# microsoft/ctsTraffic

Hardware: AMD Instinct MI355X
Metric: GiB/s verified, 64 KiB buffers device-resident; % MI355X HBM roofline (higher is better)
Workload: dtype u8

## Files before the change

ctstraffic_amd/_lib.py:

```python
from __future__ import annotations

import ctypes
import os

try:
    import torch
except Exception:
    torch = None

_HERE = os.path.dirname(os.path.abspath(__file__))
LIB_PATH = os.environ.get("CTS_ENGINE_LIB") or os.path.join(_HERE, "libcts_engine.so")

CTS_OK = 0
CTS_E_INVALID = -1
CTS_E_HIP = -2
CTS_E_NOMEM = -3
CTS_E_NO_DEVICE = -4
CTS_E_UNAVAILABLE = -5
CTS_E_TIMEOUT = -6

PATTERN_PERIOD = 65536
UDP_DATA_HEADER_LENGTH = 26
STATUS_ERROR_DATA_DID_NOT_MATCH_BIT_PATTERN = 2147483644
STATUS_ERROR_TOO_MUCH_DATA_TRANSFERRED = 2147483645
STATUS_ERROR_NOT_ALL_DATA_TRANSFERRED = 2147483646
COUNTER_SHARDS = 64
ATTR_BLOCKS_PER_CU = 1
ATTR_NT_LOADS = 2
ATTR_SMALL_THRESHOLD = 3
ATTR_VERIFY_VARIANT = 4
ATTR_SMALL_BLOCKS_PER_CU = 5
ATTR_SMALL_VARIANT = 6
ATTR_FILL_BLOCKS_PER_CU = 7
ATTR_MS_VARIANT = 8
ATTR_SMALL_CHUNK = 9
ATTR_FILL_NT = 10
ATTR_SYNC_MAILBOX = 11


VERIFY_KERNEL_ID = 25


def verify_kernel_name(nontemporal: bool = True) -> str:
    return ("void cts::verify_wg_kernel<%s>(unsigned char const*, unsigned long, cts_buf_desc const*, unsigned int, "
            "cts_verify_result*, unsigned long*, unsigned int*, unsigned int)" % ("true" if nontemporal else "false"))


class CtsError(RuntimeError):
    def __init__(self, fn: str, status: int):
        super().__init__("%s failed: %s (%d)" % (fn, _status_string(status), status))
        self.status = status


class CtsCounters(ctypes.Structure):
    _fields_ = [
        ("bytes_checked", ctypes.c_uint64),
        ("bytes_ok", ctypes.c_uint64),
        ("buffers_checked", ctypes.c_uint64),
        ("buffers_failed", ctypes.c_uint64),
        ("mismatched_bytes", ctypes.c_uint64),
    ]

    def as_dict(self) -> dict:
        return {f: int(getattr(self, f)) for f, _ in self._fields_}


class CtsCountersEx(ctypes.Structure):
    _fields_ = CtsCounters._fields_ + [("connections_failed", ctypes.c_uint64)]

    def as_dict(self) -> dict:
        return {f: int(getattr(self, f)) for f, _ in self._fields_}


class CtsCountersRef(ctypes.Structure):
    _fields_ = [
        ("bytes_recv", ctypes.c_uint64),
        ("bytes_ok", ctypes.c_uint64),
        ("buffers_recv", ctypes.c_uint64),
        ("buffers_failed", ctypes.c_uint64),
        ("bytes_after_failure", ctypes.c_uint64),
        ("buffers_after_failure", ctypes.c_uint64),
    ]

    def as_dict(self) -> dict:
        return {f: int(getattr(self, f)) for f, _ in self._fields_}


class CtsCountersClose(ctypes.Structure):
    _fields_ = [
        ("connections_closed", ctypes.c_uint64),
        ("successful", ctypes.c_uint64),
        ("data_errors", ctypes.c_uint64),
        ("not_all_data", ctypes.c_uint64),
        ("too_much_data", ctypes.c_uint64),
        ("bytes_recv", ctypes.c_uint64),
    ]

    def as_dict(self) -> dict:
        return {f: int(getattr(self, f)) for f, _ in self._fields_}


class CtsCountersUdp(ctypes.Structure):
    _fields_ = [
        ("bits_received", ctypes.c_uint64),
        ("successful_frames", ctypes.c_uint64),
        ("dropped_frames", ctypes.c_uint64),
        ("duplicate_frames", ctypes.c_uint64),
        ("error_frames", ctypes.c_uint64),
        ("datagrams", ctypes.c_uint64),
    ]

    def as_dict(self) -> dict:
        return {f: int(getattr(self, f)) for f, _ in self._fields_}


class CtsCountersSent(ctypes.Structure):
    _fields_ = [
        ("bytes_sent", ctypes.c_uint64),
        ("buffers_sent", ctypes.c_uint64),
        ("connections_finished", ctypes.c_uint64),
        ("reserved0", ctypes.c_uint64),
        ("reserved1", ctypes.c_uint64),
        ("reserved2", ctypes.c_uint64),
    ]

    def as_dict(self) -> dict:
        return {f: int(getattr(self, f)) for f, _ in self._fields_}


class CtsAllreduceSetup(ctypes.Structure):
    _fields_ = [
        ("rccl_load_ms", ctypes.c_double),
        ("slots_ms", ctypes.c_double),
        ("comm_init_ms", ctypes.c_double),
        ("first_allreduce_ms", ctypes.c_double),
        ("devices", ctypes.c_uint32),
        ("prepared", ctypes.c_uint32),
        ("last_fold_us", ctypes.c_double),
        ("last_allreduce_us", ctypes.c_double),
        ("last_readback_us", ctypes.c_double),
        ("last_total_us", ctypes.c_double),
    ]

    def as_dict(self) -> dict:
        return {f: (float if t is ctypes.c_double else int)(getattr(self, f)) for f, t in self._fields_}


class CtsVerifyResult(ctypes.Structure):
    _fields_ = [
        ("first_mismatch", ctypes.c_uint32),
        ("mismatch_bytes", ctypes.c_uint32),
        ("expected", ctypes.c_uint8),
        ("actual", ctypes.c_uint8),
        ("pass_", ctypes.c_uint8),
        ("flags", ctypes.c_uint8),
    ]


assert ctypes.sizeof(CtsVerifyResult) == 12

_lib = None


def _status_string(status: int) -> str:
    try:
        return lib().cts_status_string(status).decode()
    except Exception:
        return "status"


def _declare(L: ctypes.CDLL) -> None:
    P = ctypes.c_void_p
    u32, u64, i32 = ctypes.c_uint32, ctypes.c_uint64, ctypes.c_int
    sigs = {
        "cts_version": ([], ctypes.c_char_p),
        "cts_status_string": ([i32], ctypes.c_char_p),
        "cts_pattern_byte": ([u64], ctypes.c_uint8),
        "cts_sender_buffer_size": ([u32], u64),
        "cts_shard_of": ([u32, u32], u32),
        "cts_engine_create": ([i32, ctypes.POINTER(P)], i32),
        "cts_engine_destroy": ([P], i32),
        "cts_engine_device": ([P], i32),
        "cts_engine_numa_node": ([P], i32),
        "cts_sender_buffer_fill": ([P, P, u32, P], i32),
        "cts_fill": ([P, P, u64, P, u32, u32, P], i32),
        "cts_verify": ([P, P, u64, P, u32, u32, P, P, P, u32, P], i32),
        "cts_verify_strided": ([P, P, u64, u32, P, u32, u32, u32, u32, P, P, P, u32, P], i32),
        "cts_verify_at": ([P, P, u64, P, u32, u32, u32, P, P, P, u32, P], i32),
        "cts_verify_strided_at": ([P, P, u64, u32, P, u32, u32, u32, u32, u32, P, P, P, u32, P], i32),
        "cts_refview_accumulate": ([P, u64, P, u32, u32, P, u32, P, P], i32),
        "cts_refview_accumulate_strided": ([P, u64, u32, P, u32, u32, u32, u32, P, u32, P, P], i32),
        "cts_counters_read_ref": ([P, P, ctypes.POINTER(CtsCountersRef), P], i32),
        "cts_counters_read_multi_ref": ([ctypes.POINTER(P), ctypes.POINTER(P), ctypes.POINTER(P), u32,
                                         ctypes.POINTER(CtsCountersRef)], i32),
        "cts_counters_allreduce_ref": ([ctypes.POINTER(P), ctypes.POINTER(P), ctypes.POINTER(P), u32,
                                        ctypes.POINTER(CtsCountersRef)], i32),
        "cts_refview_accumulate_conns": ([P, u64, P, u32, u32, P, u32, P, P, P], i32),
        "cts_refview_accumulate_conns_strided": ([P, u64, u32, P, u32, u32, u32, u32, P, u32, P, P, P], i32),
        "cts_conns_close": ([P, P, P, u32, P, P, u32, P, P, P], i32),
        "cts_conn_slots_rebase": ([P, P, u32, u32, P], i32),
        "cts_counters_read_close": ([P, P, ctypes.POINTER(CtsCountersClose), P], i32),
        "cts_counters_read_multi_close": ([ctypes.POINTER(P), ctypes.POINTER(P), ctypes.POINTER(P), u32,
                                           ctypes.POINTER(CtsCountersClose)], i32),
        "cts_counters_allreduce_close": ([ctypes.POINTER(P), ctypes.POINTER(P), ctypes.POINTER(P), u32,
                                          ctypes.POINTER(CtsCountersClose)], i32),
        "cts_ms_conn_init": ([P, u64, P], i32),
        "cts_media_stream_verify_status_at": ([P, P, u64, P, u32, u32, P, P, P, u32, P], i32),
        "cts_media_stream_conns_accumulate": ([P, u64, P, P, u32, u32, P, P, P, u64, u32, P, P], i32),
        "cts_media_stream_conns_render": ([P, P, u32, P, P, u32, P, P, P], i32),
        "cts_media_stream_conns_close": ([P, P, u32, P, P, P, u32, P, P, P], i32),
        "cts_counters_read_udp": ([P, P, ctypes.POINTER(CtsCountersUdp), P], i32),
        "cts_counters_read_multi_udp": ([ctypes.POINTER(P), ctypes.POINTER(P), ctypes.POINTER(P), u32,
                                         ctypes.POINTER(CtsCountersUdp)], i32),
        "cts_counters_allreduce_udp": ([ctypes.POINTER(P), ctypes.POINTER(P), ctypes.POINTER(P), u32,
                                        ctypes.POINTER(CtsCountersUdp)], i32),
        "cts_ms_server_init": ([P, P], i32),
        "cts_media_stream_servers_scratch_bytes": ([u32], ctypes.c_size_t),
        "cts_media_stream_servers_send": ([P, P, u64, u32, u64, u32, P, u32, P, u32, ctypes.c_int64, ctypes.c_int64,
                                           P, P, P, P, P, P, ctypes.c_size_t, P], i32),
        "cts_tcp_sender_init": ([u64, u32, P], i32),
        "cts_tcp_senders_scratch_bytes": ([u32], ctypes.c_size_t),
        "cts_tcp_senders_send": ([P, P, u64, u32, u64, u32, P, u32, u32, P, u32, P, P, P, P, P, ctypes.c_size_t, P],
                                 i32),
        "cts_counters_read_sent": ([P, P, ctypes.POINTER(CtsCountersSent), P], i32),
        "cts_counters_read_multi_sent": ([ctypes.POINTER(P), ctypes.POINTER(P), ctypes.POINTER(P), u32,
                                          ctypes.POINTER(CtsCountersSent)], i32),
        "cts_counters_allreduce_sent": ([ctypes.POINTER(P), ctypes.POINTER(P), ctypes.POINTER(P), u32,
                                         ctypes.POINTER(CtsCountersSent)], i32),
        "cts_counters_device_bytes": ([], ctypes.c_size_t),
        "cts_counters_reset": ([P, P, P], i32),
        "cts_counters_read": ([P, P, ctypes.POINTER(CtsCounters), P], i32),
        "cts_counters_read_multi": ([ctypes.POINTER(P), ctypes.POINTER(P), ctypes.POINTER(P), u32,
                                     ctypes.POINTER(CtsCounters)], i32),
        "cts_counters_allreduce": ([ctypes.POINTER(P), ctypes.POINTER(P), ctypes.POINTER(P), u32,
                                    ctypes.POINTER(CtsCounters)], i32),
        "cts_counters_allreduce_release": ([], i32),
        "cts_counters_read_ex": ([P, P, ctypes.POINTER(CtsCountersEx), P], i32),
        "cts_counters_read_multi_ex": ([ctypes.POINTER(P), ctypes.POINTER(P), ctypes.POINTER(P), u32,
                                        ctypes.POINTER(CtsCountersEx)], i32),
        "cts_counters_allreduce_ex": ([ctypes.POINTER(P), ctypes.POINTER(P), ctypes.POINTER(P), u32,
                                       ctypes.POINTER(CtsCountersEx)], i32),
        "cts_counters_allreduce_prepare": ([ctypes.POINTER(P), u32], i32),
        "cts_counters_allreduce_setup_times": ([ctypes.POINTER(CtsAllreduceSetup)], i32),
        "cts_verify_host": ([P, P, u32, u32, ctypes.POINTER(CtsVerifyResult)], i32),
        "cts_verify_mapped": ([P, P, u32, u32, ctypes.POINTER(CtsVerifyResult)], i32),
        "cts_mailbox_launches": ([P], u64),
        "cts_verify_host_batch": ([P, P, P, P, P, u32, P, ctypes.POINTER(CtsCounters)], i32),
        "cts_host_alloc": ([P, u64, ctypes.POINTER(P), ctypes.POINTER(P)], i32),
        "cts_host_free": ([P, P], i32),
        "cts_engine_set_attr": ([P, i32, i32], i32),
        "cts_engine_get_attr": ([P, i32, ctypes.POINTER(i32)], i32),
        "cts_engine_stream_create": ([P, ctypes.POINTER(P)], i32),
        "cts_engine_stream_destroy": ([P, P], i32),
        "cts_host_device_pointer": ([P, ctypes.POINTER(P)], i32),
    }
    for name, (argtypes, restype) in sigs.items():
        fn = getattr(L, name)
        fn.argtypes = argtypes
        fn.restype = restype
    from . import _pattern_abi, loopback, media_stream, status

    _pattern_abi.declare(L)
    media_stream.declare(L)
    loopback.declare(L)
    status.declare(L)


def lib() -> ctypes.CDLL:
    global _lib
    if _lib is None:
        if not os.path.exists(LIB_PATH):
            raise ImportError(
                "ctstraffic_amd: %s not built — run `make` or __graft_entry__.build() "
                "(the HIP engine has no CPU fallback)" % LIB_PATH
            )
        L = ctypes.CDLL(LIB_PATH, mode=ctypes.RTLD_GLOBAL)
        _declare(L)
        _lib = L
    return _lib


def check(fn: str, status: int) -> None:
    if status != CTS_OK:
        raise CtsError(fn, status)
```

ctstraffic_amd/csrc/cts_engine.cpp:

```cpp
#include <hip/hip_runtime_api.h>

#include <algorithm>
#include <atomic>
#include <cctype>
#include <chrono>
#include <condition_variable>
#include <cstdio>
#include <cstdlib>
#include <cstring>
#include <memory>
#include <mutex>
#include <new>
#include <string>
#include <system_error>
#include <thread>
#include <vector>

#include "cts_engine.h"
#include "cts_internal.hpp"
#include "cts_slices.hpp"

struct Mailbox;

struct cts_engine {
    int device = 0;
    cts::LaunchGeometry geo;
    std::mutex host_mu;
    hipStream_t stream = nullptr;
    uint8_t* stage = nullptr;
    size_t stage_cap = 0;
    cts_buf_desc* stage_desc = nullptr;
    cts_verify_result* stage_res = nullptr;
    void* batch_desc = nullptr;
    size_t batch_desc_cap = 0;
    void* batch_res = nullptr;
    size_t batch_res_cap = 0;
    void* batch_ctr = nullptr;
    int sync_mailbox = 1;
    struct HostStage {
        void* p = nullptr;
        size_t cap = 0;
    };
    std::mutex stage_pool_mu;
    std::vector<HostStage> stage_pool;
    std::unique_ptr<Mailbox> mail;
    std::mutex mail_init_mu;
};

namespace {

int env_int(const char* name, int dflt)
{
    const char* v = std::getenv(name);
    if (v == nullptr || *v == 0) return dflt;
    return std::atoi(v);
}

struct DeviceGuard {
    int prev = -1;
    bool ok = false;
    explicit DeviceGuard(int dev)
    {
        if (hipGetDevice(&prev) != hipSuccess) prev = -1;
        ok = (prev == dev) || (hipSetDevice(dev) == hipSuccess);
    }
    ~DeviceGuard()
    {
        if (prev >= 0) (void)hipSetDevice(prev);
    }
};

inline int hip_status(hipError_t e) { return e == hipSuccess ? CTS_OK : CTS_E_HIP; }

int host_alloc_mapped(size_t bytes, void** out)
{
    void* p = nullptr;
    if (hipHostMalloc(&p, bytes, hipHostMallocMapped | hipHostMallocPortable) != hipSuccess) return CTS_E_NOMEM;
    *out = p;
    return CTS_OK;
}

template <typename T>
T* device_view(T* host)
{
    void* d = nullptr;
    if (hipHostGetDevicePointer(&d, host, 0) != hipSuccess) return nullptr;
    return static_cast<T*>(d);
}

void pinned_free(cts_engine* e, void* p);

int ensure_pinned(cts_engine* e, void** p, size_t* cap, size_t bytes, size_t floor)
{
    if (*cap >= bytes && *p != nullptr) return CTS_OK;
    if (*p) pinned_free(e, *p);
    *p = nullptr;
    *cap = 0;
    size_t c = floor;
    while (c < bytes) c <<= 1;
    const int rc = host_alloc_mapped(c, p);
    if (rc != CTS_OK) return rc;
    *cap = c;
    return CTS_OK;
}

int ensure_stage(cts_engine* e, size_t bytes)
{
    void* p = e->stage;
    const int rc = ensure_pinned(e, &p, &e->stage_cap, bytes, 1u << 20);
    e->stage = static_cast<uint8_t*>(p);
    return rc;
}

}

struct Mailbox {
    cts_engine* e = nullptr;
    uint32_t nslots = 1024, groups = 8, per_group = 128;
    int exit_ms = 1000;
    uint64_t idle_ticks = 100000000ull;
    int idle_ms = 50;
    double timeout_s = 2.0;
    uint64_t delay_ticks = 0;
    cts::MailSlot* slots = nullptr;
    cts::MailSlot* dslots = nullptr;
    cts::MailPart* parts = nullptr;
    cts::MailPart* dparts = nullptr;
    hipStream_t stream = nullptr;
    hipEvent_t grid_done = nullptr;
    std::unique_ptr<std::atomic<uint64_t>[]> free_at;
    std::mutex mu;
    bool running = false, broken = false, quit = false;
    uint32_t paused = 0;
    uint64_t next[cts::kMailMaxGroups] = {};
    uint32_t busy[cts::kMailMaxGroups] = {};
    uint32_t outstanding = 0;
    std::chrono::steady_clock::time_point last_post;
    std::chrono::steady_clock::time_point last_used[cts::kMailMaxGroups];
    std::condition_variable cv;
    std::thread watchdog;
    std::atomic<uint64_t> launches{0};
    std::atomic<bool> broken_flag{false};

    ~Mailbox();

    int Init(cts_engine* eng)
    {
        e = eng;
        nslots = (uint32_t)std::max(16, env_int("CTS_MAILBOX_SLOTS", (int)nslots));
        groups = (uint32_t)std::min((int)cts::kMailMaxGroups, std::max(1, env_int("CTS_MAILBOX_GROUPS", (int)groups)));
        idle_ms = std::max(1, env_int("CTS_MAILBOX_IDLE_MS", idle_ms));
        exit_ms = std::max(40, env_int("CTS_MAILBOX_EXIT_MS", exit_ms));
        idle_ticks = (uint64_t)exit_ms * 100000ull;
        timeout_s = std::max(1, env_int("CTS_MAILBOX_TIMEOUT_MS", (int)(timeout_s * 1000))) / 1000.0;
        delay_ticks = (uint64_t)std::max(0, env_int("CTS_MAILBOX_DELAY_MS", 0)) * 100000ull;
        DeviceGuard g(e->device);
        if (!g.ok) return CTS_E_HIP;
        void* p = nullptr;
        per_group = (nslots + groups - 1) / groups;
        nslots = per_group * groups;
        if (hipHostMalloc(&p, sizeof(cts::MailSlot) * nslots,
                          hipHostMallocMapped | hipHostMallocPortable | hipHostMallocCoherent) != hipSuccess)
            return CTS_E_NOMEM;
        slots = static_cast<cts::MailSlot*>(p);
        std::memset(slots, 0, sizeof(cts::MailSlot) * nslots);
        if ((dslots = device_view(slots)) == nullptr) return CTS_E_HIP;
        const size_t pbytes = sizeof(cts::MailPart) * nslots * cts::kMailGroup;
        if (hipHostMalloc(&p, pbytes, hipHostMallocMapped | hipHostMallocPortable | hipHostMallocCoherent) !=
            hipSuccess)
            return CTS_E_NOMEM;
        parts = static_cast<cts::MailPart*>(p);
        std::memset(parts, 0, pbytes);
        if ((dparts = device_view(parts)) == nullptr) return CTS_E_HIP;
        if (hipStreamCreateWithFlags(&stream, hipStreamNonBlocking) != hipSuccess) {
            stream = nullptr;
            return CTS_E_HIP;
        }
        if (hipEventCreateWithFlags(&grid_done, hipEventDisableTiming) != hipSuccess) {
            grid_done = nullptr;
            return CTS_E_HIP;
        }
        free_at.reset(new (std::nothrow) std::atomic<uint64_t>[nslots]);
        if (!free_at) return CTS_E_NOMEM;
        ResetRings();
        last_post = std::chrono::steady_clock::now();
        try {
            watchdog = std::thread([this] { Watch(); });
        } catch (const std::system_error&) {
            return CTS_E_NOMEM;
        }
        return CTS_OK;
    }

    void ResetRings()
    {
        std::memset(slots, 0, sizeof(cts::MailSlot) * nslots);
        std::memset(parts, 0, sizeof(cts::MailPart) * nslots * cts::kMailGroup);
        for (uint32_t i = 0; i < nslots; ++i) free_at[i].store(i % per_group, std::memory_order_relaxed);
        for (uint32_t i = 0; i < cts::kMailMaxGroups; ++i) next[i] = busy[i] = 0;
    }

    bool DrainedLocked()
    {
        if (launches.load(std::memory_order_relaxed) == 0) return true;
        DeviceGuard g(e->device);
        return hipEventQuery(grid_done) == hipSuccess;
    }

    int LaunchLocked()
    {
        DeviceGuard g(e->device);
        if (!g.ok) return CTS_E_HIP;
        cts::MailStarts starts{};
        for (uint32_t i = 0; i < groups; ++i) starts.j[i] = next[i];
        const uint64_t delay = launches.load(std::memory_order_relaxed) == 0 ? delay_ticks : 0;
        if (cts::launch_mailbox(dslots, dparts, per_group, starts, groups, idle_ticks, stream, delay) != hipSuccess ||
            hipEventRecord(grid_done, stream) != hipSuccess)
            return CTS_E_HIP;
        running = true;
        launches.fetch_add(1, std::memory_order_relaxed);
        const auto now = std::chrono::steady_clock::now();
        for (uint32_t i = 0; i < groups; ++i) last_used[i] = now;
        return CTS_OK;
    }

    int Post(uint64_t ptr, uint32_t len, uint32_t expected, cts_verify_result* out, bool only_if_idle)
    {
        uint64_t js[cts::kMailMaxGroups];
        uint32_t g0 = 0, n = 1;
        {
            std::lock_guard<std::mutex> lk(mu);
            if (broken) {
                if (len == 0 || outstanding != 0 || !DrainedLocked()) return CTS_E_HIP;
                ResetRings();
                broken = false;
                broken_flag.store(false, std::memory_order_release);
            }
            if (len != 0 && paused != 0) return CTS_E_HIP;
            if (len == 0) {
                if (!running || (only_if_idle && outstanding != 0)) return CTS_OK;
                running = false;
                if (outstanding == 0 && DrainedLocked()) return CTS_OK;
                n = groups;
            } else {
                const auto now = std::chrono::steady_clock::now();
                if (running && now - last_post > std::chrono::milliseconds(exit_ms / 2)) {
                    DeviceGuard g(e->device);
                    if (hipEventQuery(grid_done) == hipSuccess) running = false;
                }
                if (!running) {
                    const int rc = LaunchLocked();
                    if (rc != CTS_OK) return rc;
                }
                for (uint32_t i = 1; i < groups; ++i)
                    if (busy[i] < busy[g0]) g0 = i;
                for (uint32_t i = 0; i < groups; ++i)
                    if (busy[i] == 0 && now - last_used[i] > std::chrono::milliseconds(exit_ms / 4)) {
                        g0 = i;
                        break;
                    }
                last_used[g0] = now;
            }
            for (uint32_t i = 0; i < n; ++i) {
                js[i] = next[g0 + i]++;
                ++busy[g0 + i];
            }
            ++outstanding;
            last_post = std::chrono::steady_clock::now();
        }
        int rc = CTS_OK;
        for (uint32_t i = 0; i < n && rc == CTS_OK; ++i) rc = Run(g0 + i, js[i], ptr, len, expected, out);
        std::lock_guard<std::mutex> lk(mu);
        if (rc != CTS_OK) {
            broken = true;
            broken_flag.store(true, std::memory_order_release);
            running = false;
        }
        for (uint32_t i = 0; i < n; ++i) --busy[g0 + i];
        --outstanding;
        return rc;
    }

    int Run(uint32_t g, uint64_t j, uint64_t ptr, uint32_t len, uint32_t expected, cts_verify_result* out)
    {
        const uint32_t k = g * per_group + (uint32_t)(j % per_group);
        const uint64_t t = j;
        while (free_at[k].load(std::memory_order_acquire) != t) {
            if (broken_flag.load(std::memory_order_acquire)) return CTS_E_HIP;
            std::this_thread::yield();
        }
        const uint32_t tag = (uint32_t)(t + 1);
        cts::mail_write(slots + k, (ptr & 0xFFFFFFFFFFFFull) | ((uint64_t)expected << 48), (uint64_t)len | ((uint64_t)tag << 32));
        const uint32_t np = cts::mail_parts(ptr, len);
        const cts::MailPart* const pr = parts + (size_t)k * cts::kMailGroup;
        const auto t_start = std::chrono::steady_clock::now();
        uint32_t first = 0xFFFFFFFFu, actual = 0;
        uint64_t count = 0;
        for (uint32_t i = 0; i < np; ++i) {
            uint64_t g0, g1;
            for (uint32_t spin = 0;; ++spin) {
                g0 = __atomic_load_n(&pr[i].g0, __ATOMIC_ACQUIRE);
                g1 = __atomic_load_n(&pr[i].g1, __ATOMIC_ACQUIRE);
                if ((uint32_t)(g0 >> 32) == tag && (uint32_t)(g1 >> 40) == (tag & 0xFFFFFFu)) break;
                if ((spin & 255u) == 255u) {
                    if (std::chrono::duration<double>(std::chrono::steady_clock::now() - t_start).count() > timeout_s)
                        return CTS_E_HIP;
                    std::this_thread::yield();
                }
            }
            if ((uint32_t)g0 < first) {
                first = (uint32_t)g0;
                actual = (uint32_t)(g1 >> 32) & 0xFFu;
            }
            count += (uint32_t)g1;
        }
        free_at[k].store(t + per_group, std::memory_order_release);
        if (out != nullptr && len != 0) {
            const bool pass = first == 0xFFFFFFFFu;
            out->first_mismatch = pass ? len : first;
            out->mismatch_bytes = (uint32_t)count;
            out->expected = pass ? 0 : cts_pattern_byte((uint64_t)expected + first);
            out->actual = pass ? 0 : (uint8_t)actual;
            out->pass = pass ? 1 : 0;
            out->flags = 0;
        }
        return CTS_OK;
    }

    int Stop(bool only_if_idle) { return Post(0, 0, 0, nullptr, only_if_idle); }

    void Pause()
    {
        {
            std::lock_guard<std::mutex> lk(mu);
            ++paused;
        }
        (void)Stop(false);
        const auto t0 = std::chrono::steady_clock::now();
        for (;;) {
            {
                std::lock_guard<std::mutex> lk(mu);
                if (DrainedLocked()) return;
            }
            if (std::chrono::duration<double>(std::chrono::steady_clock::now() - t0).count() > timeout_s) return;
            std::this_thread::yield();
        }
    }
    void Resume()
    {
        std::lock_guard<std::mutex> lk(mu);
        --paused;
    }

    void KeepaliveLocked(std::chrono::steady_clock::time_point now)
    {
        for (uint32_t g = 0; g < groups; ++g) {
            if (busy[g] != 0 || now - last_used[g] <= std::chrono::milliseconds(exit_ms / 4)) continue;
            const uint64_t t = next[g];
            const uint32_t k = g * per_group + (uint32_t)(t % per_group);
            if (free_at[k].load(std::memory_order_acquire) != t) continue;
            ++next[g];
            cts::mail_write(slots + k, 0, (uint64_t)cts::kMailSkip | ((uint64_t)(uint32_t)(t + 1) << 32));
            free_at[k].store(t + per_group, std::memory_order_release);
            last_used[g] = now;
        }
    }

    void Watch()
    {
        std::unique_lock<std::mutex> lk(mu);
        while (!quit) {
            cv.wait_for(lk, std::chrono::milliseconds(std::max(1, std::min(idle_ms / 2, exit_ms / 8))));
            if (quit || !running || broken) continue;
            const auto now = std::chrono::steady_clock::now();
            if (now - last_post < std::chrono::milliseconds(exit_ms / 2)) KeepaliveLocked(now);
            if (outstanding != 0) continue;
            if (now - last_post < std::chrono::milliseconds(idle_ms)) continue;
            lk.unlock();
            (void)Stop(true);
            lk.lock();
        }
    }
};

namespace {

std::mutex g_mail_reg_mu;
std::vector<Mailbox*> g_mail_reg;

class DeviceQuiesce {
public:
    explicit DeviceQuiesce(int device) : dev_(device), guard_(device), lk_(g_mail_reg_mu)
    {
        for (Mailbox* m : g_mail_reg)
            if (m->e->device == dev_) m->Pause();
    }
    ~DeviceQuiesce()
    {
        for (Mailbox* m : g_mail_reg)
            if (m->e->device == dev_) m->Resume();
    }
    DeviceQuiesce(const DeviceQuiesce&) = delete;
    DeviceQuiesce& operator=(const DeviceQuiesce&) = delete;

private:
    int dev_;
    DeviceGuard guard_;
    std::unique_lock<std::mutex> lk_;
};

int pinned_free_on(int device, void* p)
{
    DeviceQuiesce q(device);
    return hip_status(hipHostFree(p));
}

void pinned_free(cts_engine* e, void* p) { (void)pinned_free_on(e->device, p); }

int mailbox_of(cts_engine* e, Mailbox** out)
{
    std::lock_guard<std::mutex> lk(e->mail_init_mu);
    if (!e->mail) {
        std::unique_ptr<Mailbox> m(new (std::nothrow) Mailbox());
        if (!m) return CTS_E_NOMEM;
        const int rc = m->Init(e);
        if (rc != CTS_OK) return rc;
        {
            std::lock_guard<std::mutex> lk(g_mail_reg_mu);
            try {
                g_mail_reg.push_back(m.get());
            } catch (const std::bad_alloc&) {
                return CTS_E_NOMEM;
            }
        }
        e->mail = std::move(m);
    }
    *out = e->mail.get();
    return CTS_OK;
}

}

Mailbox::~Mailbox()
{
    if (e == nullptr) return;
    {
        std::lock_guard<std::mutex> lk(g_mail_reg_mu);
        g_mail_reg.erase(std::remove(g_mail_reg.begin(), g_mail_reg.end(), this), g_mail_reg.end());
    }
    {
        std::lock_guard<std::mutex> lk(mu);
        quit = true;
    }
    cv.notify_all();
    if (watchdog.joinable()) watchdog.join();
    (void)Stop(false);
    {
        DeviceGuard g(e->device);
        if (stream) {
            (void)hipStreamSynchronize(stream);
            (void)hipStreamDestroy(stream);
        }
        if (grid_done) (void)hipEventDestroy(grid_done);
    }
    if (parts == nullptr && slots == nullptr) return;
    DeviceQuiesce q(e->device);
    if (parts) (void)hipHostFree(parts);
    if (slots) (void)hipHostFree(slots);
}

const cts::LaunchGeometry& cts::engine_geometry(const cts_engine* e, int* device)
{
    if (device != nullptr) *device = e->device;
    return e->geo;
}

extern "C" {

const char* cts_version(void) { return "ctstraffic_amd 0.3.0 (gfx950)"; }

const char* cts_status_string(int status)
{
    switch (status) {
    case CTS_OK: return "ok";
    case CTS_E_INVALID: return "invalid argument";
    case CTS_E_HIP: return "HIP runtime error";
    case CTS_E_NOMEM: return "out of memory";
    case CTS_E_NO_DEVICE: return "no such HIP device";
    case CTS_E_UNAVAILABLE: return "runtime library unavailable (RCCL)";
    case CTS_E_TIMEOUT: return "timed out (nothing freed; retry)";
    default: return "unknown status";
    }
}

int cts_engine_create(int device, cts_engine** out)
{
    if (out == nullptr) return CTS_E_INVALID;
    *out = nullptr;
    int count = 0;
    if (hipGetDeviceCount(&count) != hipSuccess || count <= 0) return CTS_E_NO_DEVICE;
    if (device < 0 || device >= count) return CTS_E_NO_DEVICE;
    DeviceGuard g(device);
    if (!g.ok) return CTS_E_HIP;
    cts_engine* e = new (std::nothrow) cts_engine();
    if (e == nullptr) return CTS_E_NOMEM;
    e->device = device;
    int cus = 0;
    if (hipDeviceGetAttribute(&cus, hipDeviceAttributeMultiprocessorCount, device) == hipSuccess && cus > 0)
        e->geo.num_cus = cus;
    e->geo.blocks_per_cu = env_int("CTS_BLOCKS_PER_CU", e->geo.blocks_per_cu);
    e->geo.nontemporal = env_int("CTS_NT_LOADS", e->geo.nontemporal);
    e->geo.small_threshold = env_int("CTS_SMALL_THRESHOLD", e->geo.small_threshold);
    e->geo.small_blocks_per_cu = env_int("CTS_SMALL_BLOCKS_PER_CU", e->geo.small_blocks_per_cu);
    e->geo.fill_blocks_per_cu = env_int("CTS_FILL_BLOCKS_PER_CU", e->geo.fill_blocks_per_cu);
    e->geo.small_chunk = env_int("CTS_SMALL_CHUNK", e->geo.small_chunk);
    e->geo.fill_nt = env_int("CTS_FILL_NT", e->geo.fill_nt);
    e->geo.ring_fill_blocks_per_cu = env_int("CTS_RING_FILL_BLOCKS_PER_CU", e->geo.ring_fill_blocks_per_cu);
    e->sync_mailbox = env_int("CTS_SYNC_MAILBOX", e->sync_mailbox) ? 1 : 0;
    if (hipStreamCreateWithFlags(&e->stream, hipStreamNonBlocking) != hipSuccess) {
        delete e;
        return CTS_E_HIP;
    }
    void* p = nullptr;
    if (host_alloc_mapped(cts::kSliceMax * sizeof(cts_buf_desc), &p) != CTS_OK) {
        cts_engine_destroy(e);
        return CTS_E_NOMEM;
    }
    e->stage_desc = static_cast<cts_buf_desc*>(p);
    if (host_alloc_mapped(cts::kSliceMax * sizeof(cts_verify_result), &p) != CTS_OK) {
        cts_engine_destroy(e);
        return CTS_E_NOMEM;
    }
    e->stage_res = static_cast<cts_verify_result*>(p);
    *out = e;
    return CTS_OK;
}

int cts_engine_destroy(cts_engine* e)
{
    if (e == nullptr) return CTS_E_INVALID;
    e->mail.reset();
    {
        DeviceGuard g(e->device);
        if (e->stream) {
            (void)hipStreamSynchronize(e->stream);
            (void)hipStreamDestroy(e->stream);
        }
    }
    {
        DeviceQuiesce q(e->device);
        for (auto& st : e->stage_pool) (void)hipHostFree(st.p);
        e->stage_pool.clear();
        if (e->stage) (void)hipHostFree(e->stage);
        if (e->stage_desc) (void)hipHostFree(e->stage_desc);
        if (e->stage_res) (void)hipHostFree(e->stage_res);
        if (e->batch_desc) (void)hipHostFree(e->batch_desc);
        if (e->batch_res) (void)hipHostFree(e->batch_res);
        if (e->batch_ctr) (void)hipHostFree(e->batch_ctr);
    }
    delete e;
    return CTS_OK;
}

int cts_engine_device(const cts_engine* e) { return e ? e->device : CTS_E_INVALID; }

int cts_engine_numa_node(const cts_engine* e)
{
    if (e == nullptr) return -1;
    char bus[64] = {0};
    if (hipDeviceGetPCIBusId(bus, (int)sizeof(bus), e->device) != hipSuccess) return -1;
    std::string path = "/sys/bus/pci/devices/";
    for (const char* c = bus; *c; ++c) path += (char)std::tolower((unsigned char)*c);
    path += "/numa_node";
    FILE* f = std::fopen(path.c_str(), "r");
    if (f == nullptr) return -1;
    int node = -1;
    if (std::fscanf(f, "%d", &node) != 1) node = -1;
    std::fclose(f);
    return node;
}

int cts_engine_stream_create(cts_engine* e, void** stream)
{
    if (e == nullptr || stream == nullptr) return CTS_E_INVALID;
    DeviceGuard g(e->device);
    if (!g.ok) return CTS_E_HIP;
    hipStream_t s = nullptr;
    if (hipStreamCreateWithFlags(&s, hipStreamNonBlocking) != hipSuccess) return CTS_E_HIP;
    *stream = s;
    return CTS_OK;
}

int cts_engine_stream_destroy(cts_engine* e, void* stream)
{
    if (e == nullptr || stream == nullptr) return CTS_E_INVALID;
    DeviceGuard g(e->device);
    return hip_status(hipStreamDestroy(static_cast<hipStream_t>(stream)));
}

int cts_engine_set_attr(cts_engine* e, int attr, int value)
{
    if (e == nullptr) return CTS_E_INVALID;
    switch (attr) {
    case CTS_ATTR_BLOCKS_PER_CU:
        if (value < 1 || value > 64) return CTS_E_INVALID;
        e->geo.blocks_per_cu = value;
        return CTS_OK;
    case CTS_ATTR_NT_LOADS: e->geo.nontemporal = value ? 1 : 0; return CTS_OK;
    case CTS_ATTR_SMALL_THRESHOLD:
        if (value < 0) return CTS_E_INVALID;
        e->geo.small_threshold = value;
        return CTS_OK;
    case CTS_ATTR_VERIFY_VARIANT: return value == cts::kVerifyKernelId ? CTS_OK : CTS_E_INVALID;
    case CTS_ATTR_SMALL_VARIANT: return value == cts::kSmallKernelId ? CTS_OK : CTS_E_INVALID;
    case CTS_ATTR_MS_VARIANT: return value == cts::kMediaStreamKernelId ? CTS_OK : CTS_E_INVALID;
    case CTS_ATTR_SMALL_BLOCKS_PER_CU:
        if (value < 1 || value > 256) return CTS_E_INVALID;
        e->geo.small_blocks_per_cu = value;
        return CTS_OK;
    case CTS_ATTR_FILL_BLOCKS_PER_CU:
        if (value < 1 || value > 64) return CTS_E_INVALID;
        e->geo.fill_blocks_per_cu = value;
        return CTS_OK;
    case CTS_ATTR_SMALL_CHUNK:
        if (value < 0 || value > (1 << 24)) return CTS_E_INVALID;
        e->geo.small_chunk = value;
        return CTS_OK;
    case CTS_ATTR_SYNC_MAILBOX: e->sync_mailbox = value ? 1 : 0; return CTS_OK;
    case CTS_ATTR_FILL_NT:
        if (value < 0 || value > 2) return CTS_E_INVALID;
        e->geo.fill_nt = value;
        return CTS_OK;
    default: return CTS_E_INVALID;
    }
}

int cts_engine_get_attr(const cts_engine* e, int attr, int* value)
{
    if (e == nullptr || value == nullptr) return CTS_E_INVALID;
    switch (attr) {
    case CTS_ATTR_BLOCKS_PER_CU: *value = e->geo.blocks_per_cu; return CTS_OK;
    case CTS_ATTR_NT_LOADS: *value = e->geo.nontemporal; return CTS_OK;
    case CTS_ATTR_SMALL_THRESHOLD: *value = e->geo.small_threshold; return CTS_OK;
    case CTS_ATTR_VERIFY_VARIANT: *value = cts::kVerifyKernelId; return CTS_OK;
    case CTS_ATTR_SMALL_BLOCKS_PER_CU: *value = e->geo.small_blocks_per_cu; return CTS_OK;
    case CTS_ATTR_SMALL_VARIANT: *value = cts::kSmallKernelId; return CTS_OK;
    case CTS_ATTR_FILL_BLOCKS_PER_CU: *value = e->geo.fill_blocks_per_cu; return CTS_OK;
    case CTS_ATTR_MS_VARIANT: *value = cts::kMediaStreamKernelId; return CTS_OK;
    case CTS_ATTR_SMALL_CHUNK: *value = e->geo.small_chunk; return CTS_OK;
    case CTS_ATTR_FILL_NT: *value = e->geo.fill_nt; return CTS_OK;
    case CTS_ATTR_SYNC_MAILBOX: *value = e->sync_mailbox; return CTS_OK;
    default: return CTS_E_INVALID;
    }
}

int cts_sender_buffer_fill(cts_engine* e, void* dev_dst, uint32_t max_buffer_size, void* stream)
{
    if (e == nullptr || dev_dst == nullptr || ((uintptr_t)dev_dst & 15u) != 0) return CTS_E_INVALID;
    DeviceGuard g(e->device);
    if (!g.ok) return CTS_E_HIP;
    return hip_status(cts::launch_fill_span(static_cast<uint8_t*>(dev_dst), cts_sender_buffer_size(max_buffer_size), 0,
                                            static_cast<hipStream_t>(stream), e->geo));
}

int cts_fill(cts_engine* e, void* dev_arena, uint64_t arena_bytes, const cts_buf_desc* dev_descs, uint32_t n,
             uint32_t max_length_hint, void* stream)
{
    if (e == nullptr) return CTS_E_INVALID;
    if (n == 0) return CTS_OK;
    if (dev_arena == nullptr || dev_descs == nullptr || ((uintptr_t)dev_descs & 7u) != 0 || ((uintptr_t)dev_arena & 15u) != 0) return CTS_E_INVALID;
    DeviceGuard g(e->device);
    if (!g.ok) return CTS_E_HIP;
    return hip_status(cts::launch_fill(static_cast<uint8_t*>(dev_arena), arena_bytes, dev_descs, n, max_length_hint,
                                       static_cast<hipStream_t>(stream), e->geo));
}

static bool outputs_misaligned(const void* results, const void* counters, const void* conn_first_fail = nullptr)
{
    return ((uintptr_t)results & 3u) != 0 || ((uintptr_t)counters & 7u) != 0 || ((uintptr_t)conn_first_fail & 3u) != 0;
}

int cts_verify(cts_engine* e, const void* dev_arena, uint64_t arena_bytes, const cts_buf_desc* dev_descs, uint32_t n,
               uint32_t max_length_hint, cts_verify_result* dev_results, void* dev_counters,
               uint32_t* dev_conn_first_fail, uint32_t n_conns, void* stream)
{
    if (e == nullptr) return CTS_E_INVALID;
    if (n == 0) return CTS_OK;
    if (dev_arena == nullptr || dev_descs == nullptr || ((uintptr_t)dev_descs & 7u) != 0 || ((uintptr_t)dev_arena & 15u) != 0) return CTS_E_INVALID;
    if (dev_conn_first_fail == nullptr && n_conns != 0) return CTS_E_INVALID;
    if (outputs_misaligned(dev_results, dev_counters, dev_conn_first_fail)) return CTS_E_INVALID;
    DeviceGuard g(e->device);
    if (!g.ok) return CTS_E_HIP;
    return hip_status(cts::launch_verify(static_cast<const uint8_t*>(dev_arena), arena_bytes, dev_descs, n,
                                         max_length_hint, dev_results, static_cast<uint64_t*>(dev_counters),
                                         dev_conn_first_fail, n_conns, static_cast<hipStream_t>(stream), e->geo));
}

int cts_verify_strided(cts_engine* e, const void* dev_arena, uint64_t arena_bytes, uint32_t stride,
                       const uint32_t* dev_lengths, uint32_t n, uint32_t skip_head, uint32_t expected_offset,
                       uint32_t conn_index, cts_verify_result* dev_results, void* dev_counters,
                       uint32_t* dev_conn_first_fail, uint32_t n_conns, void* stream)
{
    if (e == nullptr) return CTS_E_INVALID;
    if (n == 0) return CTS_OK;
    if (dev_arena == nullptr || dev_lengths == nullptr || stride == 0 || arena_bytes < 16 ||
        ((uintptr_t)dev_arena & 15u) != 0 || ((uintptr_t)dev_lengths & 3u) != 0)
        return CTS_E_INVALID;
    if (expected_offset >= CTS_PATTERN_PERIOD) return CTS_E_INVALID;
    if (dev_conn_first_fail == nullptr && n_conns != 0) return CTS_E_INVALID;
    if (outputs_misaligned(dev_results, dev_counters, dev_conn_first_fail)) return CTS_E_INVALID;
    DeviceGuard g(e->device);
    if (!g.ok) return CTS_E_HIP;
    return hip_status(cts::launch_verify_strided(static_cast<const uint8_t*>(dev_arena), arena_bytes, stride, dev_lengths, n,
                                                 skip_head, expected_offset, conn_index, dev_results,
                                                 static_cast<uint64_t*>(dev_counters), dev_conn_first_fail, n_conns,
                                                 static_cast<hipStream_t>(stream), e->geo));
}

int cts_media_stream_fill(cts_engine* e, void* dev_arena, uint64_t arena_bytes, const cts_buf_desc* dev_descs,
                          const cts_datagram_header* dev_headers, uint32_t n, void* stream)
{
    if (e == nullptr) return CTS_E_INVALID;
    if (n == 0) return CTS_OK;
    if (dev_arena == nullptr || dev_descs == nullptr || ((uintptr_t)dev_descs & 7u) != 0 || dev_headers == nullptr ||
        ((uintptr_t)dev_headers & 7u) != 0)
        return CTS_E_INVALID;
    DeviceGuard g(e->device);
    if (!g.ok) return CTS_E_HIP;
    return hip_status(cts::launch_media_stream_fill(static_cast<uint8_t*>(dev_arena), arena_bytes, dev_descs,
                                                    dev_headers, n, static_cast<hipStream_t>(stream), e->geo));
}

int cts_media_stream_fill_strided(cts_engine* e, void* dev_arena, uint64_t arena_bytes, uint32_t stride,
                                  const uint32_t* dev_lengths, const cts_datagram_header* dev_headers, uint32_t n,
                                  void* stream)
{
    if (e == nullptr) return CTS_E_INVALID;
    if (n == 0) return CTS_OK;
    if (dev_arena == nullptr || ((uintptr_t)dev_arena & 15u) != 0 || dev_lengths == nullptr ||
        ((uintptr_t)dev_lengths & 3u) != 0 || dev_headers == nullptr || ((uintptr_t)dev_headers & 7u) != 0 ||
        stride < 32u || (stride & 15u) != 0 || stride > (1u << 20))
        return CTS_E_INVALID;
    DeviceGuard g(e->device);
    if (!g.ok) return CTS_E_HIP;
    return hip_status(cts::launch_media_stream_fill_strided(static_cast<uint8_t*>(dev_arena), arena_bytes, stride,
                                                            dev_lengths, dev_headers, n,
                                                            static_cast<hipStream_t>(stream), e->geo));
}

int cts_media_stream_verify(cts_engine* e, const void* dev_arena, uint64_t arena_bytes, const cts_buf_desc* dev_descs,
                            uint32_t n, cts_datagram_record* dev_records, cts_verify_result* dev_results,
                            void* dev_counters, void* stream)
{
    if (e == nullptr) return CTS_E_INVALID;
    if (n == 0) return CTS_OK;
    if (dev_arena == nullptr || dev_descs == nullptr || ((uintptr_t)dev_descs & 7u) != 0 || ((uintptr_t)dev_arena & 15u) != 0) return CTS_E_INVALID;
    if (outputs_misaligned(dev_results, dev_counters, dev_records)) return CTS_E_INVALID;
    DeviceGuard g(e->device);
    if (!g.ok) return CTS_E_HIP;
    return hip_status(cts::launch_media_stream_verify(static_cast<const uint8_t*>(dev_arena), arena_bytes, dev_descs,
                                                      n, dev_records, dev_results,
                                                      static_cast<uint64_t*>(dev_counters),
                                                      static_cast<hipStream_t>(stream), e->geo));
}

int cts_media_stream_verify_strided(cts_engine* e, const void* dev_arena, uint64_t arena_bytes, uint32_t stride,
                                    const uint32_t* dev_lengths, uint32_t n, cts_datagram_record* dev_records,
                                    cts_verify_result* dev_results, void* dev_counters, void* stream)
{
    if (e == nullptr) return CTS_E_INVALID;
    if (n == 0) return CTS_OK;
    if (dev_arena == nullptr || dev_lengths == nullptr || ((uintptr_t)dev_lengths & 3u) != 0 ||
        ((uintptr_t)dev_arena & 15u) != 0 || arena_bytes < 16u || stride == 0)
        return CTS_E_INVALID;
    if (outputs_misaligned(dev_results, dev_counters, dev_records)) return CTS_E_INVALID;
    DeviceGuard g(e->device);
    if (!g.ok) return CTS_E_HIP;
    return hip_status(cts::launch_media_stream_verify_strided(static_cast<const uint8_t*>(dev_arena), arena_bytes, stride,
                                                              dev_lengths, n, dev_records, dev_results,
                                                              static_cast<uint64_t*>(dev_counters),
                                                              static_cast<hipStream_t>(stream), e->geo));
}

int cts_media_stream_verify_status(cts_engine* e, const void* dev_arena, uint64_t arena_bytes,
                                   const cts_buf_desc* dev_descs, uint32_t n, cts_datagram_status* dev_status,
                                   void* dev_counters, void* stream)
{
    if (e == nullptr) return CTS_E_INVALID;
    if (n == 0) return CTS_OK;
    if (dev_arena == nullptr || dev_descs == nullptr || ((uintptr_t)dev_descs & 7u) != 0 || ((uintptr_t)dev_arena & 15u) != 0 ||
        outputs_misaligned(dev_status, dev_counters))
        return CTS_E_INVALID;
    DeviceGuard g(e->device);
    if (!g.ok) return CTS_E_HIP;
    return hip_status(cts::launch_media_stream_status(static_cast<const uint8_t*>(dev_arena), arena_bytes, dev_descs,
                                                      nullptr, 0u, n, dev_status, static_cast<uint64_t*>(dev_counters),
                                                      static_cast<hipStream_t>(stream), e->geo));
}

int cts_media_stream_verify_strided_status(cts_engine* e, const void* dev_arena, uint64_t arena_bytes, uint32_t stride,
                                           const uint32_t* dev_lengths, uint32_t n, cts_datagram_status* dev_status,
                                           void* dev_counters, void* stream)
{
    if (e == nullptr) return CTS_E_INVALID;
    if (n == 0) return CTS_OK;
    if (dev_arena == nullptr || dev_lengths == nullptr || ((uintptr_t)dev_lengths & 3u) != 0 ||
        ((uintptr_t)dev_arena & 15u) != 0 || arena_bytes < 16u || stride == 0 || outputs_misaligned(dev_status, dev_counters))
        return CTS_E_INVALID;
    DeviceGuard g(e->device);
    if (!g.ok) return CTS_E_HIP;
    return hip_status(cts::launch_media_stream_status(static_cast<const uint8_t*>(dev_arena), arena_bytes, nullptr,
                                                      dev_lengths, stride, n, dev_status,
                                                      static_cast<uint64_t*>(dev_counters),
                                                      static_cast<hipStream_t>(stream), e->geo));
}

static int media_stream_frames(cts_engine* e, const void* dev_arena, uint64_t arena_bytes, const cts_buf_desc* dev_descs,
                               uint32_t stride, const uint32_t* dev_lengths, uint32_t n, const cts_frame_window* w,
                               void* dev_totals, uint64_t* dev_frame_bytes, void* dev_counters, void* stream)
{
    if (e == nullptr || w == nullptr || dev_totals == nullptr || ((uintptr_t)dev_totals & 7u) != 0 ||
        (w->frames != 0 && (dev_frame_bytes == nullptr || ((uintptr_t)dev_frame_bytes & 7u) != 0)))
        return CTS_E_INVALID;
    if (n != 0 && (dev_arena == nullptr || ((uintptr_t)dev_arena & 15u) != 0 || outputs_misaligned(nullptr, dev_counters)))
        return CTS_E_INVALID;
    if (n != 0 && dev_descs == nullptr &&
        (dev_lengths == nullptr || ((uintptr_t)dev_lengths & 3u) != 0 || arena_bytes < 16u || stride == 0))
        return CTS_E_INVALID;
    if (n != 0 && dev_descs != nullptr && ((uintptr_t)dev_descs & 7u) != 0) return CTS_E_INVALID;
    DeviceGuard g(e->device);
    if (!g.ok) return CTS_E_HIP;
    return hip_status(cts::launch_media_stream_frames(static_cast<const uint8_t*>(dev_arena), arena_bytes, dev_descs,
                                                      dev_lengths, stride, n, *w, static_cast<uint64_t*>(dev_totals),
                                                      dev_frame_bytes, static_cast<uint64_t*>(dev_counters),
                                                      static_cast<hipStream_t>(stream), e->geo));
}

int cts_media_stream_verify_frames(cts_engine* e, const void* dev_arena, uint64_t arena_bytes,
                                   const cts_buf_desc* dev_descs, uint32_t n, const cts_frame_window* window,
                                   void* dev_totals, uint64_t* dev_frame_bytes, void* dev_counters, void* stream)
{
    if (n != 0 && dev_descs == nullptr) return CTS_E_INVALID;
    return media_stream_frames(e, dev_arena, arena_bytes, dev_descs, 0u, nullptr, n, window, dev_totals,
                               dev_frame_bytes, dev_counters, stream);
}

int cts_media_stream_verify_strided_frames(cts_engine* e, const void* dev_arena, uint64_t arena_bytes, uint32_t stride,
                                           const uint32_t* dev_lengths, uint32_t n, const cts_frame_window* window,
                                           void* dev_totals, uint64_t* dev_frame_bytes, void* dev_counters,
                                           void* stream)
{
    if (n != 0 && dev_lengths == nullptr) return CTS_E_INVALID;
    return media_stream_frames(e, dev_arena, arena_bytes, nullptr, stride, dev_lengths, n, window, dev_totals,
                               dev_frame_bytes, dev_counters, stream);
}

size_t cts_counters_device_bytes(void) { return (size_t)CTS_COUNTER_SHARDS * cts::kCounterSlots * sizeof(uint64_t); }

int cts_counters_reset(cts_engine* e, void* dev_counters, void* stream)
{
    if (e == nullptr || dev_counters == nullptr) return CTS_E_INVALID;
    DeviceGuard g(e->device);
    if (!g.ok) return CTS_E_HIP;
    return hip_status(hipMemsetAsync(dev_counters, 0, cts_counters_device_bytes(), static_cast<hipStream_t>(stream)));
}

int cts_counters_read_ex(cts_engine* e, const void* dev_counters, cts_counters_ex* out, void* stream)
{
    if (e == nullptr || dev_counters == nullptr || out == nullptr) return CTS_E_INVALID;
    DeviceGuard g(e->device);
    if (!g.ok) return CTS_E_HIP;
    uint64_t h[CTS_COUNTER_SHARDS * cts::kCounterSlots];
    hipStream_t s = static_cast<hipStream_t>(stream);
    if (hipMemcpyAsync(h, dev_counters, cts_counters_device_bytes(), hipMemcpyDeviceToHost, s) != hipSuccess)
        return CTS_E_HIP;
    if (hipStreamSynchronize(s) != hipSuccess) return CTS_E_HIP;
    uint64_t v[cts::kCounterCount] = {};
    for (uint32_t sh = 0; sh < CTS_COUNTER_SHARDS; ++sh)
        for (int k = 0; k < cts::kCounterCount; ++k) v[k] += h[sh * cts::kCounterSlots + k];
    *out = cts::counters_ex_of(v);
    return CTS_OK;
}

int cts_counters_read(cts_engine* e, const void* dev_counters, cts_counters* out, void* stream)
{
    if (out == nullptr) return CTS_E_INVALID;
    cts_counters_ex x{};
    const int rc = cts_counters_read_ex(e, dev_counters, &x, stream);
    if (rc == CTS_OK) *out = cts::counters_of(x);
    return rc;
}

int cts_host_alloc(cts_engine* e, uint64_t bytes, void** host_ptr, void** dev_view)
{
    if (e == nullptr || host_ptr == nullptr || bytes == 0) return CTS_E_INVALID;
    DeviceGuard g(e->device);
    if (!g.ok) return CTS_E_HIP;
    void* p = nullptr;
    const int rc = host_alloc_mapped((size_t)((bytes + 15u) & ~(uint64_t)15u), &p);
    if (rc != CTS_OK) return rc;
    *host_ptr = p;
    if (dev_view != nullptr) {
        void* d = nullptr;
        if (hipHostGetDevicePointer(&d, p, 0) != hipSuccess) {
            (void)pinned_free_on(e->device, p);
            *host_ptr = nullptr;
            return CTS_E_HIP;
        }
        *dev_view = d;
    }
    return CTS_OK;
}

int cts_host_free(cts_engine* e, void* host_ptr)
{
    if (e == nullptr || host_ptr == nullptr) return CTS_E_INVALID;
    return pinned_free_on(e->device, host_ptr);
}

int cts_host_device_pointer(void* host_ptr, void** dev_view)
{
    if (host_ptr == nullptr || dev_view == nullptr) return CTS_E_INVALID;
    void* d = nullptr;
    if (hipHostGetDevicePointer(&d, host_ptr, 0) != hipSuccess) return CTS_E_INVALID;
    *dev_view = d;
    return CTS_OK;
}

int cts_verify_host(cts_engine* e, const void* host_buf, uint32_t len, uint32_t expected_offset, cts_verify_result* out)
{
    if (e == nullptr || out == nullptr || (host_buf == nullptr && len != 0)) return CTS_E_INVALID;
    if (expected_offset >= CTS_PATTERN_PERIOD) return CTS_E_INVALID;
    if (e->sync_mailbox) {
        cts_engine::HostStage st;
        {
            std::lock_guard<std::mutex> lk(e->stage_pool_mu);
            if (!e->stage_pool.empty()) {
                st = e->stage_pool.back();
                e->stage_pool.pop_back();
            }
        }
        int rc = ensure_pinned(e, &st.p, &st.cap, (size_t)len + 16, 64u << 10);
        const uint8_t* dev = rc == CTS_OK ? device_view(static_cast<uint8_t*>(st.p)) : nullptr;
        if (rc == CTS_OK && dev == nullptr) rc = CTS_E_HIP;
        if (rc == CTS_OK) {
            if (len) std::memcpy(st.p, host_buf, len);
            rc = cts_verify_mapped(e, dev, len, expected_offset, out);
        }
        if (st.p != nullptr) {
            bool pooled = false;
            {
                std::lock_guard<std::mutex> lk(e->stage_pool_mu);
                try {
                    e->stage_pool.push_back(st);
                    pooled = true;
                } catch (const std::bad_alloc&) {
                }
            }
            if (!pooled) pinned_free(e, st.p);
        }
        return rc;
    }
    std::lock_guard<std::mutex> lk(e->host_mu);
    DeviceGuard g(e->device);
    if (!g.ok) return CTS_E_HIP;
    int rc = ensure_stage(e, (size_t)len + 16);
    if (rc != CTS_OK) return rc;
    if (len) std::memcpy(e->stage, host_buf, len);
    uint32_t slice_len = 0;
    const uint32_t ns = cts::slice_plan(0, len, expected_offset, 0, e->stage_desc, &slice_len);
    const uint8_t* arena = device_view(e->stage);
    const cts_buf_desc* dd = device_view(e->stage_desc);
    cts_verify_result* dr = device_view(e->stage_res);
    if (!arena || !dd || !dr) return CTS_E_HIP;
    hipError_t err = cts::launch_verify(arena, e->stage_cap, dd, ns, slice_len, dr, nullptr, nullptr, 0, e->stream,
                                        e->geo);
    if (err == hipSuccess) err = hipStreamSynchronize(e->stream);
    if (err != hipSuccess) return CTS_E_HIP;
    *out = cts::slice_merge(e->stage_res, ns, slice_len, len);
    return CTS_OK;
}

int cts_verify_host_batch(cts_engine* e, const void* const* bufs, const uint32_t* lens, const uint32_t* expected,
                          const uint32_t* skip_heads, uint32_t n, cts_verify_result* results, cts_counters* counters)
{
    if (e == nullptr) return CTS_E_INVALID;
    if (n == 0) return CTS_OK;
    if (bufs == nullptr || lens == nullptr || expected == nullptr || results == nullptr) return CTS_E_INVALID;
    std::lock_guard<std::mutex> lk(e->host_mu);
    DeviceGuard g(e->device);
    if (!g.ok) return CTS_E_HIP;
    uint64_t total = 0;
    for (uint32_t i = 0; i < n; ++i) {
        if (bufs[i] == nullptr && lens[i] != 0) return CTS_E_INVALID;
        total += ((uint64_t)lens[i] + 15u) & ~(uint64_t)15u;
    }
    int rc = ensure_stage(e, (size_t)total + 16);
    if (rc != CTS_OK) return rc;
    if ((rc = ensure_pinned(e, &e->batch_desc, &e->batch_desc_cap, sizeof(cts_buf_desc) * n, 4096)) != CTS_OK) return rc;
    if ((rc = ensure_pinned(e, &e->batch_res, &e->batch_res_cap, sizeof(cts_verify_result) * n, 4096)) != CTS_OK) return rc;
    if (counters && e->batch_ctr == nullptr &&
        (rc = host_alloc_mapped(cts_counters_device_bytes(), &e->batch_ctr)) != CTS_OK)
        return rc;
    void* const pres = e->batch_res;
    void* const pctr = counters ? e->batch_ctr : nullptr;
    cts_buf_desc* hd = static_cast<cts_buf_desc*>(e->batch_desc);
    uint64_t off = 0;
    uint32_t maxlen = 0;
    for (uint32_t i = 0; i < n; ++i) {
        if (lens[i]) std::memcpy(e->stage + off, bufs[i], lens[i]);
        hd[i].byte_offset = off;
        hd[i].length = lens[i];
        hd[i].expected_pattern_offset = expected[i];
        hd[i].conn_index = i;
        hd[i].skip_head = skip_heads ? skip_heads[i] : 0u;
        maxlen = lens[i] > maxlen ? lens[i] : maxlen;
        off += ((uint64_t)lens[i] + 15u) & ~(uint64_t)15u;
    }
    if (pctr) std::memset(pctr, 0, cts_counters_device_bytes());
    hipError_t err = cts::launch_verify(device_view(e->stage), e->stage_cap, device_view(hd), n, maxlen,
                                        device_view(static_cast<cts_verify_result*>(pres)),
                                        pctr ? device_view(static_cast<uint64_t*>(pctr)) : nullptr, nullptr, 0,
                                        e->stream, e->geo);
    if (err == hipSuccess) err = hipStreamSynchronize(e->stream);
    if (err == hipSuccess) {
        std::memcpy(results, pres, sizeof(cts_verify_result) * n);
        if (counters) {
            const uint64_t* h = static_cast<const uint64_t*>(pctr);
            for (uint32_t sh = 0; sh < CTS_COUNTER_SHARDS; ++sh) {
                counters->bytes_checked += h[sh * cts::kCounterSlots + cts::kBytesChecked];
                counters->bytes_ok += h[sh * cts::kCounterSlots + cts::kBytesOk];
                counters->buffers_checked += h[sh * cts::kCounterSlots + cts::kBuffersChecked];
                counters->buffers_failed += h[sh * cts::kCounterSlots + cts::kBuffersFailed];
                counters->mismatched_bytes += h[sh * cts::kCounterSlots + cts::kMismatchedBytes];
            }
        }
    }
    return err == hipSuccess ? CTS_OK : CTS_E_HIP;
}

int cts_verify_mapped(cts_engine* e, const void* dev_buf, uint32_t len, uint32_t expected_offset,
                      cts_verify_result* out)
{
    if (e == nullptr || out == nullptr || (dev_buf == nullptr && len != 0)) return CTS_E_INVALID;
    if (expected_offset >= CTS_PATTERN_PERIOD) return CTS_E_INVALID;
    if (len == 0) {
        *out = cts_verify_result{0, 0, 0, 0, 1, 0};
        return CTS_OK;
    }
    Mailbox* m = nullptr;
    const int rc = mailbox_of(e, &m);
    if (rc != CTS_OK) return rc;
    if (m->Post(reinterpret_cast<uint64_t>(dev_buf), len, expected_offset, out, false) == CTS_OK) return CTS_OK;
    std::lock_guard<std::mutex> lk(e->host_mu);
    DeviceGuard g(e->device);
    if (!g.ok) return CTS_E_HIP;
    const uint64_t d = reinterpret_cast<uintptr_t>(dev_buf) & 15u;
    uint32_t slice_len = 0;
    const uint32_t ns = cts::slice_plan(d, len, expected_offset, 0, e->stage_desc, &slice_len);
    const cts_buf_desc* dd = device_view(e->stage_desc);
    cts_verify_result* dr = device_view(e->stage_res);
    if (!dd || !dr) return CTS_E_HIP;
    hipError_t err = cts::launch_verify(static_cast<const uint8_t*>(dev_buf) - d, d + len, dd, ns, slice_len, dr,
                                        nullptr, nullptr, 0, e->stream, e->geo);
    if (err == hipSuccess) err = hipStreamSynchronize(e->stream);
    if (err != hipSuccess) return CTS_E_HIP;
    *out = cts::slice_merge(e->stage_res, ns, slice_len, len);
    return CTS_OK;
}

uint64_t cts_mailbox_launches(const cts_engine* e)
{
    return (e != nullptr && e->mail) ? e->mail->launches.load(std::memory_order_relaxed) : 0;
}

}
```

ctstraffic_amd/csrc/cts_fill.hip:

```cpp
#include <hip/hip_runtime.h>

#include "cts_chunks.hpp"
#include "cts_launch.hpp"

namespace cts {


__device__ __forceinline__ void store_chunk_bytes(uint8_t* dst, const u32x4& e, uint32_t b0, uint32_t b1)
{
#pragma unroll
    for (uint32_t w = 0; w < 4u; ++w) {
        const uint32_t lo = b0 > 4u * w ? b0 - 4u * w : 0u, hi = b1 < 4u * w + 4u ? (b1 > 4u * w ? b1 - 4u * w : 0u) : 4u;
        if (lo >= hi) continue;
        uint8_t* q = dst + 4u * w;
        const uint32_t v = e[w];
        if (lo == 0u && hi == 4u) {
            *reinterpret_cast<uint32_t*>(q) = v;
            continue;
        }
        uint32_t b = lo;
        if ((b & 1u) && b < hi) {
            q[b] = (uint8_t)(v >> (8u * b));
            ++b;
        }
        if (b + 2u <= hi) {
            *reinterpret_cast<uint16_t*>(q + b) = (uint16_t)(v >> (8u * b));
            b += 2u;
        }
        if (b < hi) q[b] = (uint8_t)(v >> (8u * b));
    }
}

template <bool NTS = false>
__device__ __forceinline__ void fill_chunk(u32x4* a0, uint32_t c, uint32_t nchunks, uint32_t q0, uint32_t lo,
                                           uint32_t hi_last)
{
    const u32x4 e = expected_chunk((q0 + 16u * c) & 0xFFFFu, q0 & 1u);
    const bool first_c = (c == 0u);
    const bool last_c = (c == nchunks - 1u);
    const uint32_t b0 = first_c ? lo : 0u;
    const uint32_t b1 = last_c ? hi_last : 16u;
    if (b0 == 0u && b1 == 16u) {
        if constexpr (NTS) __builtin_nontemporal_store(e, a0 + c);
        else a0[c] = e;
    } else {
        store_chunk_bytes(reinterpret_cast<uint8_t*>(a0 + c), e, b0, b1);
    }
}

template <int TEAM, int U, bool EVEN, bool NTS>
__device__ __forceinline__ void fill_whole_rounds(u32x4* p, uint32_t nchunks, uint32_t q0, uint32_t lane)
{
    const uint32_t sh = q0 & 1u;
    typedef u32x4 __attribute__((address_space(1)))* gstore_ptr;
    uint32_t cb = 0;
    for (; cb + (uint32_t)(TEAM * U) <= nchunks; cb += (uint32_t)(TEAM * U)) {
        const uint32_t k = ((q0 + 16u * (cb + lane)) & 0xFFFFu) >> 1;
        const uint32_t B = __umul24(k, 0x10001u) + 0x10000u;
        const gstore_ptr g = (gstore_ptr)(p + cb + lane);
#pragma unroll
        for (int u = 0; u < U; ++u) {
            const u32x4 e = expected_step<TEAM, U, EVEN>(B, u, sh);
            if constexpr (NTS) __builtin_nontemporal_store(e, g + u * TEAM);
            else g[u * TEAM] = e;
        }
    }
    if (cb < nchunks) {
        const __amdgpu_buffer_rsrc_t r = __builtin_amdgcn_make_buffer_rsrc(p, (short)0, (int)(nchunks * 16u), 0x00020000);
        const uint32_t k = ((q0 + 16u * (cb + lane)) & 0xFFFFu) >> 1;
        const uint32_t B = __umul24(k, 0x10001u) + 0x10000u;
#pragma unroll
        for (int u = 0; u < U; ++u)
            __builtin_amdgcn_raw_buffer_store_b128(expected_step<TEAM, U, EVEN>(B, u, sh), r,
                                                   (cb + (uint32_t)(u * TEAM) + lane) * 16u, 0u, NTS ? 2 : 0);
    }
}

template <int TEAM, int FU, bool NTS>
__device__ __forceinline__ void fill_one(uint8_t* arena, uint64_t arena_bytes, const cts_buf_desc& d, uint32_t lane)
{
    if (desc_bad(d, arena_bytes)) return;
    const uint32_t len = d.length - d.skip_head;
    if (len == 0) return;
    uint8_t* sp = arena + d.byte_offset + d.skip_head;
    const uint32_t lo = (uint32_t)((uintptr_t)sp & 15u);
    const uint32_t nchunks = (uint32_t)(((uint64_t)lo + len + 15u) >> 4);
    const uint32_t hi_last = (uint32_t)((uint64_t)lo + len - 16ull * (nchunks - 1u));
    const uint32_t q0 = (d.expected_pattern_offset - lo) & 0xFFFFu;
    u32x4* p = reinterpret_cast<u32x4*>(sp - lo);
    if (__builtin_amdgcn_readfirstlane((lo == 0u && hi_last == 16u && nchunks < kGiantChunks) ? 1u : 0u)) {
        if (__builtin_amdgcn_readfirstlane(q0 & 1u) == 0u) fill_whole_rounds<TEAM, FU, true, NTS>(p, nchunks, q0, lane);
        else fill_whole_rounds<TEAM, FU, false, NTS>(p, nchunks, q0, lane);
        return;
    }
    for (uint32_t c = lane; c < nchunks; c += TEAM) fill_chunk<NTS>(p, c, nchunks, q0, lo, hi_last);
}

template <int TEAM, bool NTS = false>
__global__ void __launch_bounds__(kBlock) fill_kernel(uint8_t* __restrict__ arena, uint64_t arena_bytes,
                                                      const cts_buf_desc* __restrict__ descs, uint32_t n)
{
#include "cts_fill_team_loop.hpp"
}

constexpr uint32_t kFillPiece = 8192;
constexpr int kPieceBatch = 16;

struct PieceJob {
    uint64_t base;
    uint32_t q0;
    uint32_t cb, ce;
    uint32_t nchunks, lo, hi_last;
    uint32_t kind;
};

template <uint32_t PIECE>
__device__ __forceinline__ PieceJob decode_piece(uint8_t* arena, uint64_t arena_bytes, const cts_buf_desc* descs,
                                                 uint64_t v, uint64_t total, uint32_t ppb, bool mine)
{
    constexpr uint32_t kChunks = PIECE / 16;
    PieceJob j{};
    if (!mine || v >= total) return j;
    const uint32_t i = (uint32_t)(v / ppb), pc = (uint32_t)(v - (uint64_t)i * ppb);
    const cts_buf_desc d = descs[i];
    if (desc_bad(d, arena_bytes) || d.length == d.skip_head) return j;
    const uint32_t len = d.length - d.skip_head;
    const uint64_t sp = (uint64_t)(uintptr_t)arena + d.byte_offset + d.skip_head;
    j.lo = (uint32_t)(sp & 15u);
    j.nchunks = (uint32_t)(((uint64_t)j.lo + len + 15u) >> 4);
    j.hi_last = (uint32_t)((uint64_t)j.lo + len - 16ull * (j.nchunks - 1u));
    j.q0 = (d.expected_pattern_offset - j.lo) & 0xFFFFu;
    j.base = sp - j.lo;
    const uint64_t cb = (uint64_t)pc * kChunks;
    if (cb >= j.nchunks) return j;
    j.cb = (uint32_t)cb;
    j.ce = pc + 1u == ppb ? j.nchunks : (uint32_t)(cb + kChunks < j.nchunks ? cb + kChunks : j.nchunks);
    j.kind = (j.lo == 0u && j.hi_last == 16u) ? 1u : 2u;
    return j;
}

__device__ __forceinline__ uint32_t lane_u32(uint32_t x, int m) { return (uint32_t)__builtin_amdgcn_readlane((int)x, m); }

template <bool NTS, uint32_t PIECE = kFillPiece, int BATCH = kPieceBatch>
__global__ void __launch_bounds__(kBlock) fill_pieces_kernel(uint8_t* __restrict__ arena, uint64_t arena_bytes,
                                                             const cts_buf_desc* __restrict__ descs, uint32_t n,
                                                             uint32_t ppb)
{
#include "cts_fill_pieces_loop.hpp"
}

__global__ void __launch_bounds__(kBlock) fill_span_kernel(uint8_t* __restrict__ dst, uint64_t bytes, uint32_t e)
{
    const uint32_t lo = (uint32_t)((uintptr_t)dst & 15u);
    const uint32_t nchunks = (uint32_t)((lo + bytes + 15u) >> 4);
    const uint32_t hi_last = (uint32_t)(lo + bytes - 16ull * (nchunks - 1u));
    const uint32_t q0 = (e - lo) & 0xFFFFu;
    u32x4* p = reinterpret_cast<u32x4*>(dst - lo);
    for (uint32_t c = blockIdx.x * kBlock + threadIdx.x; c < nchunks; c += gridDim.x * kBlock)
        fill_chunk(p, c, nchunks, q0, lo, hi_last);
}

template <bool NTS>
__device__ __forceinline__ void ms_fill_one(uint8_t* arena, uint64_t arena_bytes, const cts_buf_desc& d, uint64_t seq,
                                            uint64_t qpc, uint64_t qpf, uint32_t lane)
{
    if (d.length < CTS_UDP_DATA_HEADER_LENGTH || d.byte_offset > arena_bytes ||
        arena_bytes - d.byte_offset < (uint64_t)d.length)
        return;
    uint8_t* dg = arena + d.byte_offset;
    if (__builtin_amdgcn_readfirstlane(((uintptr_t)dg & 15u) == 0u ? 1u : 0u)) {
        const uint32_t nchunks = (d.length + 15u) >> 4;
        const uint32_t hi_last = d.length - 16u * (nchunks - 1u);
        u32x4* p = reinterpret_cast<u32x4*>(dg);
        for (uint32_t c = lane; c < nchunks; c += 64u) {
            u32x4 e = expected_chunk((16u * c - CTS_UDP_DATA_HEADER_LENGTH) & 0xFFFFu, 0u);
            if (c == 0u)
                e = u32x4{(uint32_t)(seq << 16), (uint32_t)(seq >> 16), (uint32_t)(seq >> 48) | (uint32_t)(qpc << 16),
                          (uint32_t)(qpc >> 16)};
            else if (c == 1u)
                e = u32x4{(uint32_t)(qpc >> 48) | (uint32_t)(qpf << 16), (uint32_t)(qpf >> 16),
                          (uint32_t)(qpf >> 48) | (e[2] & 0xFFFF0000u), e[3]};
            if (c == nchunks - 1u && hi_last != 16u) {
                store_chunk_bytes(reinterpret_cast<uint8_t*>(p + c), e, 0u, hi_last);
            } else {
                if constexpr (NTS) __builtin_nontemporal_store(e, p + c);
                else p[c] = e;
            }
        }
        return;
    }
    if (lane < CTS_UDP_DATA_HEADER_LENGTH) {
        uint8_t b = 0;
        if (lane >= 2u && lane < 10u) b = (uint8_t)(seq >> (8 * (lane - 2u)));
        else if (lane >= 10u && lane < 18u) b = (uint8_t)(qpc >> (8 * (lane - 10u)));
        else if (lane >= 18u) b = (uint8_t)(qpf >> (8 * (lane - 18u)));
        dg[lane] = b;
    }
    const uint32_t len = d.length - CTS_UDP_DATA_HEADER_LENGTH;
    if (len == 0) return;
    uint8_t* sp = dg + CTS_UDP_DATA_HEADER_LENGTH;
    const uint32_t lo = (uint32_t)((uintptr_t)sp & 15u);
    const uint32_t nchunks = (uint32_t)(((uint64_t)lo + len + 15u) >> 4);
    const uint32_t hi_last = (uint32_t)((uint64_t)lo + len - 16ull * (nchunks - 1u));
    const uint32_t q0 = (0u - lo) & 0xFFFFu;
    u32x4* p = reinterpret_cast<u32x4*>(sp - lo);
    for (uint32_t c = lane; c < nchunks; c += 64u) fill_chunk<NTS>(p, c, nchunks, q0, lo, hi_last);
}

constexpr uint32_t kFillBatch = kBlock;

template <bool NTS>
__global__ void __launch_bounds__(kBlock)
    fill_batched_kernel(uint8_t* __restrict__ arena, uint64_t arena_bytes, const cts_buf_desc* __restrict__ descs,
                        const cts_datagram_header* __restrict__ headers, uint32_t n)
{
    constexpr uint32_t WAVES = kBlock / 64;
    __shared__ cts_buf_desc ds[kFillBatch];
    __shared__ cts_datagram_header hs[kFillBatch];
    const uint32_t lane = threadIdx.x & 63u;
    const uint32_t wave = (uint32_t)__builtin_amdgcn_readfirstlane(threadIdx.x >> 6);
    const uint32_t per_wg = (uint32_t)(((uint64_t)n + gridDim.x - 1u) / gridDim.x);
    const uint64_t g0 = (uint64_t)blockIdx.x * per_wg;
    const uint64_t g1 = g0 + per_wg < n ? g0 + per_wg : n;
    for (uint64_t d0 = g0; d0 < g1; d0 += kFillBatch) {
        const uint32_t nb = (uint32_t)(g1 - d0 < kFillBatch ? g1 - d0 : kFillBatch);
        __syncthreads();
        if (threadIdx.x < nb) {
            ds[threadIdx.x] = descs[d0 + threadIdx.x];
            hs[threadIdx.x] = headers[d0 + threadIdx.x];
        }
        __syncthreads();
        const uint32_t q = (nb + WAVES - 1u) / WAVES;
        const uint32_t t1 = (wave + 1u) * q < nb ? (wave + 1u) * q : nb;
        for (uint32_t t = wave * q; t < t1; ++t) {
            const cts_datagram_header h = hs[t];
            ms_fill_one<NTS>(arena, arena_bytes, ds[t], (uint64_t)h.sequence_number, (uint64_t)h.qpc, (uint64_t)h.qpf,
                             lane);
        }
    }
}


constexpr uint32_t kRingBatch = 512;

struct RingHeader {
    uint64_t seq, qpc, qpf;
};

__device__ __forceinline__ u32x4 datagram_chunk(uint32_t c, const u32x4& pattern, uint64_t seq, uint64_t qpc,
                                                uint64_t qpf)
{
    if (c == 0u)
        return u32x4{(uint32_t)(seq << 16), (uint32_t)(seq >> 16), (uint32_t)(seq >> 48) | (uint32_t)(qpc << 16),
                     (uint32_t)(qpc >> 16)};
    if (c == 1u)
        return u32x4{(uint32_t)(qpc >> 48) | (uint32_t)(qpf << 16), (uint32_t)(qpf >> 16),
                     (uint32_t)(qpf >> 48) | (pattern[2] & 0xFFFF0000u), pattern[3]};
    return pattern;
}

__device__ __forceinline__ u32x4 header_lanes(u32x4 e, uint32_t lane, uint32_t l0, const RingHeader& h)
{
    if (lane == l0) {
        e = u32x4{(uint32_t)(h.seq << 16), (uint32_t)(h.seq >> 16), (uint32_t)(h.seq >> 48) | (uint32_t)(h.qpc << 16),
                  (uint32_t)(h.qpc >> 16)};
    } else if (lane == l0 + 1u) {
        e[0] = (uint32_t)(h.qpc >> 48) | (uint32_t)(h.qpf << 16);
        e[1] = (uint32_t)(h.qpf >> 16);
        e[2] = (uint32_t)(h.qpf >> 48) | (e[2] & 0xFFFF0000u);
    }
    return e;
}

template <bool NTS>
__device__ __forceinline__ void ring_chunk_checked(u32x4* ring, uint64_t k, uint64_t j, uint32_t c, uint32_t len,
                                                   const RingHeader& h, uint32_t stride, uint64_t arena_bytes)
{
    if (len < CTS_UDP_DATA_HEADER_LENGTH || len > stride || 16u * c >= len || j * stride + len > arena_bytes) return;
    const u32x4 e = datagram_chunk(c, expected_chunk((16u * c - CTS_UDP_DATA_HEADER_LENGTH) & 0xFFFFu, 0u), h.seq,
                                   h.qpc, h.qpf);
    if (16u * c + 16u > len) {
        store_chunk_bytes(reinterpret_cast<uint8_t*>(ring + k), e, 0u, len - 16u * c);
    } else {
        if constexpr (NTS) __builtin_nontemporal_store(e, ring + k);
        else ring[k] = e;
    }
}

template <bool NTS, bool SCALAR>
__global__ void __launch_bounds__(kBlock)
    media_stream_fill_ring_kernel(uint8_t* __restrict__ arena, uint64_t arena_bytes, uint32_t stride,
                                  const uint32_t* __restrict__ lengths, const cts_datagram_header* __restrict__ headers,
                                  uint32_t n, uint32_t full_slots)
{
    constexpr uint32_t WAVES = kBlock / 64;
    __shared__ RingHeader hs[kRingBatch];
    __shared__ uint32_t ls[kRingBatch];
    const uint32_t lane = threadIdx.x & 63u;
    const uint32_t wave = (uint32_t)__builtin_amdgcn_readfirstlane(threadIdx.x >> 6);
    const uint32_t cps = stride >> 4;
    const uint32_t per_wg = (uint32_t)(((uint64_t)n + gridDim.x - 1u) / gridDim.x);
    const uint64_t g0 = (uint64_t)blockIdx.x * per_wg;
    const uint64_t g1 = g0 + per_wg < n ? g0 + per_wg : n;
    u32x4* const ring = reinterpret_cast<u32x4*>(arena);
    for (uint64_t d0 = g0; d0 < g1; d0 += kRingBatch) {
        const uint32_t nb = (uint32_t)(g1 - d0 < kRingBatch ? g1 - d0 : kRingBatch);
        __syncthreads();
        for (uint32_t t = threadIdx.x; t < nb; t += kBlock) {
            const cts_datagram_header h = headers[d0 + t];
            hs[t] = RingHeader{(uint64_t)h.sequence_number, (uint64_t)h.qpc, (uint64_t)h.qpf};
            ls[t] = lengths[d0 + t];
        }
        __syncthreads();
#include "cts_ring_store_loop.hpp"
    }
}


__device__ __forceinline__ uint32_t ms_server_want(const cts_ms_server_state* __restrict__ servers, uint32_t c,
                                                   uint32_t n_conns, uint32_t stride, uint32_t& code)
{
    code = CTS_MS_SERVER_SKIPPED;
    if (c >= n_conns) return 0u;
    if (servers[c].finished != 0u) {
        code = CTS_MS_SERVER_ENDED;
        return 0u;
    }
    if (servers[c].datagram_max_size > stride) return 0u;
    code = CTS_MS_SERVER_SENT;
    return servers[c].datagrams_per_frame;
}

__device__ __forceinline__ uint64_t tile_scan_exclusive(uint64_t v, uint64_t* wsum, uint64_t& total)
{
    const uint32_t lane = threadIdx.x & 63u, wave = threadIdx.x >> 6;
    uint64_t inc = v;
#pragma unroll
    for (uint32_t off = 1; off < 64u; off <<= 1) {
        const uint64_t u = (uint64_t)__shfl_up((unsigned long long)inc, off, 64);
        if (lane >= off) inc += u;
    }
    if (lane == 63u) wsum[wave] = inc;
    __syncthreads();
    uint64_t base = 0;
    total = 0;
#pragma unroll
    for (uint32_t w = 0; w < (uint32_t)kBlock / 64u; ++w) {
        if (w < wave) base += wsum[w];
        total += wsum[w];
    }
    __syncthreads();
    return base + inc - v;
}

static_assert(kMsServerTile == (uint32_t)kBlock, "one listed connection per thread of a tile");

__global__ void __launch_bounds__(kBlock)
    ms_server_sums(const uint32_t* __restrict__ ids, uint32_t n, const cts_ms_server_state* __restrict__ servers,
                   uint32_t n_conns, uint32_t stride, uint64_t* __restrict__ sums)
{
    __shared__ uint64_t wsum[kBlock / 64];
    const uint64_t i = (uint64_t)blockIdx.x * kMsServerTile + threadIdx.x;
    uint32_t code;
    const uint64_t want = i < n ? ms_server_want(servers, ids[i], n_conns, stride, code) : 0u;
    const uint64_t s = wave_sum64(want);
    if ((threadIdx.x & 63u) == 0u) wsum[threadIdx.x >> 6] = s;
    __syncthreads();
    if (threadIdx.x == 0u) {
        uint64_t t = 0;
#pragma unroll
        for (int w = 0; w < kBlock / 64; ++w) t += wsum[w];
        sums[blockIdx.x] = t;
    }
}

__global__ void __launch_bounds__(kBlock)
    ms_server_scan(uint64_t* __restrict__ sums, uint64_t tiles, uint64_t* __restrict__ prefix_total,
                   uint32_t* __restrict__ tick)
{
    __shared__ uint64_t wsum[kBlock / 64];
    uint64_t carry = 0;
    for (uint64_t base = 0; base < tiles; base += kBlock) {
        const uint64_t t = base + threadIdx.x;
        const uint64_t v = t < tiles ? sums[t] : 0u;
        uint64_t total;
        const uint64_t ex = tile_scan_exclusive(v, wsum, total);
        if (t < tiles) sums[t] = carry + ex;
        carry += total;
    }
    if (threadIdx.x == 0u) *prefix_total = carry;
    if (threadIdx.x < sizeof(cts_ms_server_tick) / 4u) tick[threadIdx.x] = 0u;
}

__global__ void __launch_bounds__(kBlock)
    ms_server_apply(const uint32_t* __restrict__ ids, uint32_t n, cts_ms_server_state* __restrict__ servers,
                    uint32_t n_conns, uint32_t stride, uint32_t capacity, const uint64_t* __restrict__ sums,
                    uint64_t* __restrict__ prefix, uint32_t* __restrict__ codes, cts_ms_server_tick* __restrict__ tick,
                    uint64_t* __restrict__ udp)
{
    __shared__ uint64_t wsum[kBlock / 64];
    __shared__ uint64_t ctr[kBlock / 64][kCounterCount];
    __shared__ uint32_t red[kBlock / 64][5];
    zero_counters<kBlock / 64>(ctr);
    const uint64_t i = (uint64_t)blockIdx.x * kMsServerTile + threadIdx.x;
    uint32_t code = CTS_MS_SERVER_SENT, c = 0u;
    uint64_t want = 0;
    if (i < n) {
        c = ids[i];
        want = ms_server_want(servers, c, n_conns, stride, code);
    }
    uint64_t total;
    const uint64_t p = sums[blockIdx.x] + tile_scan_exclusive(want, wsum, total);
    uint64_t bytes = 0;
    uint32_t datagrams = 0, sent = 0, finished = 0, no_room = 0, skipped = 0;
    if (i < n) {
        prefix[i] = p;
        if (code != CTS_MS_SERVER_SENT) {
            skipped = 1u;
        } else if (p + want > (uint64_t)capacity) {
            no_room = 1u;
            code = CTS_MS_SERVER_NO_ROOM;
        } else {
            cts_ms_server_state* e = servers + c;
            bytes = e->frame_size_bytes;
            datagrams = (uint32_t)want;
            sent = 1u;
            e->bits_sent += 8u * bytes;
            e->datagrams_sent += want;
            const int64_t next = e->current_frame + 1;
            e->current_frame = next;
            if (next > e->final_frame) {
                e->finished = 1u;
                finished = 1u;
                code = CTS_MS_SERVER_FINISHED;
            }
        }
        if (codes != nullptr) codes[i] = code;
    }
    bytes = wave_sum64(bytes);
    datagrams = wave_sum(datagrams);
    sent = wave_sum(sent);
    finished = wave_sum(finished);
    no_room = wave_sum(no_room);
    skipped = wave_sum(skipped);
    const uint32_t wave = threadIdx.x >> 6;
    if ((threadIdx.x & 63u) == 0u) {
        ctr[wave][0] = 8u * bytes;
        ctr[wave][kCounterCount - 1] = datagrams;
        red[wave][0] = datagrams;
        red[wave][1] = sent;
        red[wave][2] = finished;
        red[wave][3] = no_room;
        red[wave][4] = skipped;
    }
    flush_counters<kBlock / 64>(udp, ctr);
    if (threadIdx.x < 5u) {
        uint32_t s = 0;
#pragma unroll
        for (int w = 0; w < kBlock / 64; ++w) s += red[w][threadIdx.x];
        uint32_t* const words = &tick->datagrams;
        if (s) atomicAdd(words + threadIdx.x, s);
    } else if (threadIdx.x == 5u) {
        uint64_t s = 0;
#pragma unroll
        for (int w = 0; w < kBlock / 64; ++w) s += ctr[w][0];
        if (s) atomicAdd((unsigned long long*)&tick->bytes, (unsigned long long)(s / 8u));
    }
}

__device__ __forceinline__ uint64_t ms_server_listed(const uint64_t* __restrict__ prefix, uint64_t lo, uint64_t hi,
                                                     uint64_t g)
{
    while (hi - lo > 1u) {
        const uint64_t mid = lo + (hi - lo) / 2u;
        if (prefix[mid] <= g) lo = mid;
        else hi = mid;
    }
    return lo;
}

__device__ __forceinline__ uint32_t ms_server_length(uint32_t F, uint32_t M, uint32_t k, uint32_t j)
{
    const uint32_t r = F % (M != 0u ? M : 1u);
    const bool tiny = r != 0u && r <= CTS_UDP_DATA_HEADER_LENGTH;
    if (j + 1u == k) return r == 0u ? M : (tiny && k > 1u ? CTS_UDP_DATA_HEADER_LENGTH + 1u : r);
    if (j + 2u == k && tiny) return M - (CTS_UDP_DATA_HEADER_LENGTH + 1u - r);
    return M;
}

template <bool NTS, bool SCALAR>
__global__ void __launch_bounds__(kBlock)
    ms_server_fill(uint8_t* __restrict__ ring_base, uint64_t arena_bytes, uint32_t stride, uint64_t first_slot,
                          const uint32_t* __restrict__ ids, uint32_t n,
                          const cts_ms_server_state* __restrict__ servers, const uint64_t* __restrict__ prefix,
                          const cts_ms_server_tick* __restrict__ tick, uint64_t qpc, uint64_t qpf,
                          cts_buf_desc* __restrict__ descs, uint32_t* __restrict__ lengths, uint32_t full_slots,
                          uint32_t capacity, uint32_t n_conns)
{
    constexpr uint32_t WAVES = kBlock / 64;
    __shared__ RingHeader hs[kRingBatch];
    __shared__ uint32_t ls[kRingBatch];
    __shared__ uint64_t ps[kRingBatch + 1];
    __shared__ uint64_t first_listed;
    const uint32_t total = tick->datagrams < capacity ? tick->datagrams : capacity;
    if (total == 0u) return;
    const uint32_t lane = threadIdx.x & 63u;
    const uint32_t wave = (uint32_t)__builtin_amdgcn_readfirstlane(threadIdx.x >> 6);
    const uint32_t cps = stride >> 4;
    const uint32_t even = (uint32_t)(((uint64_t)total + gridDim.x - 1u) / gridDim.x);
    const uint32_t least = total < kRingBatch ? total : kRingBatch;
    const uint32_t per_wg = even > least ? even : least;
    const uint64_t g0 = (uint64_t)blockIdx.x * per_wg;
    if (g0 >= total) return;
    const uint64_t g1 = g0 + per_wg < total ? g0 + per_wg : total;
    if (threadIdx.x == 0u) first_listed = ms_server_listed(prefix, 0u, n, g0);
    u32x4* const ring = reinterpret_cast<u32x4*>(ring_base);
    for (uint64_t d0 = g0; d0 < g1; d0 += kRingBatch) {
        const uint32_t nb = (uint32_t)(g1 - d0 < kRingBatch ? g1 - d0 : kRingBatch);
        __syncthreads();
        const uint64_t i0 = first_listed;
        for (uint32_t t = threadIdx.x; t <= kRingBatch; t += kBlock) ps[t] = prefix[i0 + t < n ? i0 + t : n];
        __syncthreads();
        for (uint32_t t = threadIdx.x; t < nb; t += kBlock) {
            const uint64_t g = d0 + t;
            uint32_t lo = 0u, hi = kRingBatch + 1u;
            while (hi - lo > 1u) {
                const uint32_t mid = (lo + hi) >> 1;
                if (ps[mid] <= g) lo = mid;
                else hi = mid;
            }
            uint64_t i = i0 + lo, p = ps[lo];
            if (lo == kRingBatch && i + 1u < n) {
                i = ms_server_listed(prefix, i, n, g);
                p = prefix[i];
            }
            if (i >= n) i = n - 1u;
            const uint32_t c = ids[i];
            const cts_ms_server_state* e = servers + (c < n_conns ? c : 0u);
            const uint32_t len = c >= n_conns ? 0u
                                              : ms_server_length(e->frame_size_bytes, e->datagram_max_size,
                                                                 e->datagrams_per_frame, (uint32_t)(g - p));
            hs[t] = RingHeader{(uint64_t)(e->current_frame - 1), qpc, qpf};
            ls[t] = len;
            if (descs != nullptr)
                descs[g] = cts_buf_desc{(first_slot + g) * stride, len, 0u, c, CTS_UDP_DATA_HEADER_LENGTH};
            if (lengths != nullptr) lengths[g] = len;
            if (t == nb - 1u) first_listed = i;
        }
        __syncthreads();
#include "cts_ring_store_loop.hpp"
    }
}

static_assert(sizeof(cts_tcp_sender_tick) == sizeof(cts_ms_server_tick), "ms_server_scan zeroes either tick block");

__device__ __forceinline__ uint64_t tcp_sender_want(const cts_tcp_sender_state* __restrict__ senders, uint32_t c,
                                                    uint32_t n_conns, uint32_t stride, uint32_t max_buffers,
                                                    uint32_t& code)
{
    code = CTS_TCP_SENDER_SKIPPED;
    if (c >= n_conns) return 0u;
    const uint32_t B = senders[c].buffer_size;
    if (B == 0u || B > stride) return 0u;
    code = CTS_TCP_SENDER_ENDED;
    const uint64_t sent = senders[c].bytes_sent, transfer = senders[c].transfer_bytes;
    if (senders[c].finished != 0u || sent >= transfer) return 0u;
    code = CTS_TCP_SENDER_SENT;
    const uint64_t R = transfer - sent;
    const uint64_t k = R / B + (R % B != 0u ? 1u : 0u);
    return k < max_buffers ? k : max_buffers;
}

__device__ __forceinline__ uint64_t tcp_wave_sum64(uint64_t v)
{
    uint64_t s = 0;
#pragma unroll
    for (int l = 0; l < 4; ++l) s += (uint64_t)wave_sum((uint32_t)(v >> (16 * l)) & 0xFFFFu) << (16 * l);
    return s;
}

__global__ void __launch_bounds__(kBlock)
    tcp_sender_sums(const uint32_t* __restrict__ ids, uint32_t n, const cts_tcp_sender_state* __restrict__ senders,
                    uint32_t n_conns, uint32_t stride, uint32_t max_buffers, uint64_t* __restrict__ sums)
{
    __shared__ uint64_t wsum[kBlock / 64];
    const uint64_t i = (uint64_t)blockIdx.x * kMsServerTile + threadIdx.x;
    uint32_t code;
    const uint64_t want = i < n ? tcp_sender_want(senders, ids[i], n_conns, stride, max_buffers, code) : 0u;
    const uint64_t s = tcp_wave_sum64(want);
    if ((threadIdx.x & 63u) == 0u) wsum[threadIdx.x >> 6] = s;
    __syncthreads();
    if (threadIdx.x == 0u) {
        uint64_t t = 0;
#pragma unroll
        for (int w = 0; w < kBlock / 64; ++w) t += wsum[w];
        sums[blockIdx.x] = t;
    }
}

__global__ void __launch_bounds__(kBlock)
    tcp_sender_apply(const uint32_t* __restrict__ ids, uint32_t n, cts_tcp_sender_state* __restrict__ senders,
                     uint32_t n_conns, uint32_t stride, uint32_t capacity, uint32_t max_buffers,
                     const uint64_t* __restrict__ sums, uint64_t* __restrict__ prefix, uint64_t* __restrict__ before,
                     uint32_t* __restrict__ codes, cts_tcp_sender_tick* __restrict__ tick, uint64_t* __restrict__ sent_block)
{
    __shared__ uint64_t wsum[kBlock / 64];
    __shared__ uint64_t ctr[kBlock / 64][kCounterCount];
    __shared__ uint32_t red[kBlock / 64][5];
    zero_counters<kBlock / 64>(ctr);
    const uint64_t i = (uint64_t)blockIdx.x * kMsServerTile + threadIdx.x;
    uint32_t code = CTS_TCP_SENDER_SENT, c = 0u;
    uint64_t want = 0;
    if (i < n) {
        c = ids[i];
        want = tcp_sender_want(senders, c, n_conns, stride, max_buffers, code);
    }
    uint64_t total;
    const uint64_t p = sums[blockIdx.x] + tile_scan_exclusive(want, wsum, total);
    uint64_t bytes = 0;
    uint32_t buffers = 0, sent = 0, finished = 0, no_room = 0, skipped = 0;
    if (i < n) {
        prefix[i] = p;
        const uint64_t pc = p < (uint64_t)capacity ? p : (uint64_t)capacity;
        const uint64_t t = want < (uint64_t)capacity - pc ? want : (uint64_t)capacity - pc;
        uint64_t was = 0;
        if (code != CTS_TCP_SENDER_SENT) {
            skipped = 1u;
        } else if (t == 0u) {
            no_room = 1u;
            code = CTS_TCP_SENDER_NO_ROOM;
        } else {
            cts_tcp_sender_state* e = senders + c;
            was = e->bytes_sent;
            const uint64_t R = e->transfer_bytes - was, full = t * e->buffer_size;
            bytes = full < R ? full : R;
            buffers = (uint32_t)t;
            sent = 1u;
            e->bytes_sent = was + bytes;
            e->buffers_sent += t;
            if (bytes == R) {
                e->finished = 1u;
                finished = 1u;
                code = CTS_TCP_SENDER_FINISHED;
            }
        }
        before[i] = was;
        if (codes != nullptr) codes[i] = code;
    }
    const uint64_t own_bytes = tcp_wave_sum64(bytes);
    buffers = wave_sum(buffers);
    sent = wave_sum(sent);
    finished = wave_sum(finished);
    no_room = wave_sum(no_room);
    skipped = wave_sum(skipped);
    const uint32_t wave = threadIdx.x >> 6;
    if ((threadIdx.x & 63u) == 0u) {
        ctr[wave][0] = own_bytes;
        ctr[wave][1] = buffers;
        ctr[wave][2] = finished;
        red[wave][0] = buffers;
        red[wave][1] = sent;
        red[wave][2] = finished;
        red[wave][3] = no_room;
        red[wave][4] = skipped;
    }
    flush_counters<kBlock / 64>(sent_block, ctr);
    if (threadIdx.x < 5u) {
        uint32_t s = 0;
#pragma unroll
        for (int w = 0; w < kBlock / 64; ++w) s += red[w][threadIdx.x];
        uint32_t* const words = &tick->buffers;
        if (s) atomicAdd(words + threadIdx.x, s);
    } else if (threadIdx.x == 5u) {
        uint64_t s = 0;
#pragma unroll
        for (int w = 0; w < kBlock / 64; ++w) s += ctr[w][0];
        if (s) atomicAdd((unsigned long long*)&tick->bytes, (unsigned long long)s);
    }
}

__global__ void __launch_bounds__(kBlock)
    tcp_sender_descs(uint32_t stride, uint64_t first_slot, uint32_t capacity, const uint32_t* __restrict__ ids,
                     uint32_t n, const cts_tcp_sender_state* __restrict__ senders, uint32_t n_conns,
                     const uint64_t* __restrict__ prefix, const uint64_t* __restrict__ before,
                     const cts_tcp_sender_tick* __restrict__ tick, cts_buf_desc* __restrict__ descs)
{
    const uint32_t total = tick->buffers < capacity ? tick->buffers : capacity;
    for (uint64_t g = (uint64_t)blockIdx.x * kBlock + threadIdx.x; g < total; g += (uint64_t)gridDim.x * kBlock) {
        const uint64_t i = ms_server_listed(prefix, 0u, n, g);
        const uint64_t j = g - prefix[i];
        const uint32_t c = ids[i];
        uint32_t len = 0u, off = 0u;
        if (c < n_conns) {
            const uint32_t B = senders[c].buffer_size;
            const uint64_t was = before[i], start = was + j * B;
            const uint64_t end = senders[c].transfer_bytes;
            const uint64_t left = start < end ? end - start : 0u;
            len = left < (uint64_t)B ? (uint32_t)left : B;
            if (len > stride) len = 0u;
            off = (uint32_t)(start & 0xFFFFu);
        }
        descs[g] = cts_buf_desc{(first_slot + g) * stride, len, off, c, 0u};
    }
}

template <bool NTS>
__global__ void __launch_bounds__(kBlock)
    tcp_sender_fill_pieces(uint8_t* __restrict__ arena, uint64_t arena_bytes, const cts_buf_desc* __restrict__ descs,
                           const cts_tcp_sender_tick* __restrict__ tick, uint32_t capacity, uint32_t ppb)
{
    constexpr uint32_t PIECE = kFillPiece;
    constexpr int BATCH = kPieceBatch;
    const uint32_t n = tick->buffers < capacity ? tick->buffers : capacity;
#include "cts_fill_pieces_loop.hpp"
}

template <bool NTS>
__global__ void __launch_bounds__(kBlock)
    tcp_sender_fill_small(uint8_t* __restrict__ arena, uint64_t arena_bytes, const cts_buf_desc* __restrict__ descs,
                          const cts_tcp_sender_tick* __restrict__ tick, uint32_t capacity)
{
    constexpr int TEAM = 64;
    const uint32_t n = tick->buffers < capacity ? tick->buffers : capacity;
#include "cts_fill_team_loop.hpp"
}

static_assert(kGridBlock == (uint32_t)kBlock && kGridFillPiece == kFillPiece && kGridFillBatch == kFillBatch &&
                  kGridRingBatch == kRingBatch,
              "cts_grids.hpp sizes the launches of these kernels");

hipError_t launch_fill(uint8_t* arena, uint64_t arena_bytes, const cts_buf_desc* descs, uint32_t n,
                       uint32_t max_length_hint, hipStream_t stream, const LaunchGeometry& geo)
{
    if (n == 0) return hipSuccess;
    const bool small = max_length_hint != 0 && max_length_hint <= (uint32_t)geo.small_threshold;
    const bool nts = geo.fill_nt == 2 ? small : geo.fill_nt != 0;
    with_flags(
        [&](auto NTS) {
            if (!small && max_length_hint != 0) {
                const PieceGrid pg = piece_fill_grid(n, max_length_hint, geo.num_cus, geo.fill_blocks_per_cu);
                fill_pieces_kernel<NTS.value><<<pg.grid, kBlock, 0, stream>>>(arena, arena_bytes, descs, n, pg.ppb);
            } else if (small) {
                fill_kernel<64, NTS.value><<<grid_for(n, kBlock / 64, geo), kBlock, 0, stream>>>(arena, arena_bytes,
                                                                                                 descs, n);
            } else {
                fill_kernel<kBlock, NTS.value><<<grid_for(n, 1, geo, geo.fill_blocks_per_cu), kBlock, 0, stream>>>(
                    arena, arena_bytes, descs, n);
            }
        },
        nts);
    return hipGetLastError();
}

hipError_t launch_media_stream_fill(uint8_t* arena, uint64_t arena_bytes, const cts_buf_desc* descs,
                                   const cts_datagram_header* headers, uint32_t n, hipStream_t stream,
                                   const LaunchGeometry& geo)
{
    if (n == 0) return hipSuccess;
    const uint32_t grid = batched_fill_grid(n, geo.num_cus, geo.ring_fill_blocks_per_cu);
    with_flags(
        [&](auto NTS) {
            fill_batched_kernel<NTS.value><<<grid, kBlock, 0, stream>>>(arena, arena_bytes, descs, headers, n);
        },
        geo.fill_nt == 1);
    return hipGetLastError();
}

hipError_t launch_media_stream_fill_strided(uint8_t* arena, uint64_t arena_bytes, uint32_t stride, const uint32_t* lengths,
                                           const cts_datagram_header* headers, uint32_t n, hipStream_t stream,
                                           const LaunchGeometry& geo)
{
    if (n == 0) return hipSuccess;
    if ((stride & 15u) != 0u || stride < 32u || stride > (1u << 20) || ((uintptr_t)arena & 15u) != 0u)
        return hipErrorInvalidValue;
    const uint32_t grid = ring_fill_grid(n, geo.num_cus, geo.ring_fill_blocks_per_cu);
    const uint64_t slots = arena_bytes / stride;
    const uint32_t full_slots = (uint32_t)(slots < 0xFFFFFFFFull ? slots : 0xFFFFFFFFull);
    with_flags(
        [&](auto NTS, auto SCALAR) {
            media_stream_fill_ring_kernel<NTS.value, SCALAR.value><<<grid, kBlock, 0, stream>>>(
                arena, arena_bytes, stride, lengths, headers, n, full_slots);
        },
        geo.fill_nt != 0, stride >= 1024u);
    return hipGetLastError();
}

hipError_t launch_ms_server_plan(const uint32_t* conn_ids, uint32_t n, cts_ms_server_state* servers, uint32_t n_conns,
                                 uint32_t stride, uint32_t capacity, uint32_t* codes, cts_ms_server_tick* tick,
                                 uint64_t* udp_counters, const MsServerScratch& scratch, hipStream_t stream)
{
    if (n == 0) return hipSuccess;
    const uint64_t tiles = ms_server_tiles(n);
    ms_server_sums<<<(uint32_t)tiles, kBlock, 0, stream>>>(conn_ids, n, servers, n_conns, stride, scratch.sums);
    ms_server_scan<<<1, kBlock, 0, stream>>>(scratch.sums, tiles, scratch.prefix + n,
                                             reinterpret_cast<uint32_t*>(tick));
    ms_server_apply<<<(uint32_t)tiles, kBlock, 0, stream>>>(conn_ids, n, servers, n_conns, stride, capacity,
                                                            scratch.sums, scratch.prefix, codes, tick, udp_counters);
    return hipGetLastError();
}

hipError_t launch_ms_server_fill(uint8_t* arena, uint64_t arena_bytes, uint32_t stride, uint64_t first_slot,
                                 uint32_t capacity, const uint32_t* conn_ids, uint32_t n,
                                 const cts_ms_server_state* servers, uint32_t n_conns, const uint64_t* prefix,
                                 const cts_ms_server_tick* tick, int64_t qpc, int64_t qpf, cts_buf_desc* descs,
                                 uint32_t* lengths, hipStream_t stream, const LaunchGeometry& geo)
{
    if (n == 0 || capacity == 0) return hipSuccess;
    if ((stride & 15u) != 0u || stride < 32u || stride > (1u << 20) || ((uintptr_t)arena & 15u) != 0u ||
        first_slot > arena_bytes / stride)
        return hipErrorInvalidValue;
    const uint32_t grid = ring_fill_grid(capacity, geo.num_cus, geo.ring_fill_blocks_per_cu);
    uint8_t* const ring = arena + first_slot * stride;
    const uint64_t ring_bytes = arena_bytes - first_slot * stride;
    const uint64_t slots = ring_bytes / stride;
    const uint32_t full_slots = (uint32_t)(slots < 0xFFFFFFFFull ? slots : 0xFFFFFFFFull);
    with_flags(
        [&](auto NTS, auto SCALAR) {
            ms_server_fill<NTS.value, SCALAR.value><<<grid, kBlock, 0, stream>>>(
                ring, ring_bytes, stride, first_slot, conn_ids, n, servers, prefix, tick, (uint64_t)qpc, (uint64_t)qpf,
                descs, lengths, full_slots, capacity, n_conns);
        },
        geo.fill_nt != 0, stride >= 1024u);
    return hipGetLastError();
}

hipError_t launch_tcp_sender_plan(const uint32_t* conn_ids, uint32_t n, uint32_t max_buffers,
                                  cts_tcp_sender_state* senders, uint32_t n_conns, uint32_t stride, uint32_t capacity,
                                  uint32_t* codes, cts_tcp_sender_tick* tick, uint64_t* sent_counters,
                                  const TcpSenderScratch& scratch, hipStream_t stream)
{
    if (n == 0) return hipSuccess;
    const uint64_t tiles = ms_server_tiles(n);
    tcp_sender_sums<<<(uint32_t)tiles, kBlock, 0, stream>>>(conn_ids, n, senders, n_conns, stride, max_buffers,
                                                            scratch.sums);
    ms_server_scan<<<1, kBlock, 0, stream>>>(scratch.sums, tiles, scratch.prefix + n,
                                             reinterpret_cast<uint32_t*>(tick));
    tcp_sender_apply<<<(uint32_t)tiles, kBlock, 0, stream>>>(conn_ids, n, senders, n_conns, stride, capacity,
                                                             max_buffers, scratch.sums, scratch.prefix, scratch.before,
                                                             codes, tick, sent_counters);
    return hipGetLastError();
}

hipError_t launch_tcp_sender_descs(uint32_t stride, uint64_t first_slot, uint32_t capacity, const uint32_t* conn_ids,
                                   uint32_t n, const cts_tcp_sender_state* senders, uint32_t n_conns,
                                   const TcpSenderScratch& scratch, const cts_tcp_sender_tick* tick,
                                   cts_buf_desc* descs, hipStream_t stream, const LaunchGeometry& geo)
{
    if (n == 0 || capacity == 0) return hipSuccess;
    const uint32_t grid = grid_for((uint32_t)(((uint64_t)capacity + kBlock - 1) / kBlock), 1, geo);
    tcp_sender_descs<<<grid, kBlock, 0, stream>>>(stride, first_slot, capacity, conn_ids, n, senders, n_conns,
                                                  scratch.prefix, scratch.before, tick, descs);
    return hipGetLastError();
}

hipError_t launch_tcp_sender_fill(uint8_t* arena, uint64_t arena_bytes, uint32_t stride, uint32_t capacity,
                                  const cts_buf_desc* descs, const cts_tcp_sender_tick* tick, hipStream_t stream,
                                  const LaunchGeometry& geo)
{
    if (capacity == 0) return hipSuccess;
    const bool small = stride <= (uint32_t)geo.small_threshold;
    const bool nts = geo.fill_nt == 2 ? small : geo.fill_nt != 0;
    with_flags(
        [&](auto NTS) {
            if (!small) {
                const PieceGrid pg = piece_fill_grid(capacity, stride, geo.num_cus, geo.fill_blocks_per_cu);
                tcp_sender_fill_pieces<NTS.value><<<pg.grid, kBlock, 0, stream>>>(arena, arena_bytes, descs, tick,
                                                                                 capacity, pg.ppb);
            } else {
                tcp_sender_fill_small<NTS.value><<<grid_for(capacity, kBlock / 64, geo), kBlock, 0, stream>>>(
                    arena, arena_bytes, descs, tick, capacity);
            }
        },
        nts);
    return hipGetLastError();
}

hipError_t launch_fill_span(uint8_t* dst, uint64_t bytes, uint32_t pattern_offset, hipStream_t stream,
                            const LaunchGeometry& geo)
{
    if (bytes == 0) return hipSuccess;
    const uint64_t chunks = (bytes + 30) / 16 + 1;
    const uint32_t grid = grid_for((uint32_t)((chunks + kBlock - 1) / kBlock), 1, geo);
    fill_span_kernel<<<grid, kBlock, 0, stream>>>(dst, bytes, pattern_offset & 0xFFFFu);
    return hipGetLastError();
}

}
```

ctstraffic_amd/csrc/cts_grids.hpp:

```cpp
#pragma once

#include <stdint.h>

namespace cts {

constexpr uint32_t kGridBlock = 256;
constexpr uint32_t kGridQuadTeams = 16;
constexpr uint32_t kGridFillPiece = 8192;
constexpr uint32_t kGridFillBatch = 256;
constexpr uint32_t kGridRingBatch = 512;

inline uint32_t grid_for(uint32_t n, int teams_per_block, int num_cus, int bpc)
{
    const uint64_t want = ((uint64_t)n + teams_per_block - 1) / teams_per_block;
    const uint64_t cap = (uint64_t)num_cus * (uint64_t)(bpc > 0 ? bpc : 8);
    const uint64_t per = want <= cap ? 1 : (want + cap - 1) / cap;
    const uint64_t g = (want + per - 1) / per;
    return (uint32_t)(g == 0 ? 1 : g);
}

struct ContigGrid {
    uint32_t grid, per;
};
inline ContigGrid contig_grid(uint32_t n, int num_cus, int small_bpc, int small_chunk)
{
    const uint32_t teams = kGridQuadTeams;
    const uint32_t g = grid_for(n, (int)teams, num_cus, small_bpc);
    if (small_chunk > 0) {
        const uint64_t per = ((uint64_t)small_chunk + teams - 1) / teams * teams;
        const uint64_t chunks = ((uint64_t)n + per - 1) / per;
        return ContigGrid{(uint32_t)(chunks < g ? chunks : g), (uint32_t)per};
    }
    const uint64_t groups = ((uint64_t)n + teams - 1) / teams;
    const uint64_t per = (groups + g - 1) / g * teams;
    return ContigGrid{(uint32_t)(((uint64_t)n + per - 1) / per), (uint32_t)per};
}

inline uint32_t batch_fill_grid(uint32_t n, uint32_t batch, int num_cus, int ring_bpc)
{
    const uint64_t cap = (uint64_t)num_cus * (uint64_t)(ring_bpc > 0 ? ring_bpc : 4);
    const uint64_t want = ((uint64_t)n + batch - 1) / batch;
    return (uint32_t)(want < cap ? want : cap);
}
inline uint32_t batched_fill_grid(uint32_t n, int num_cus, int ring_bpc)
{
    return batch_fill_grid(n, kGridFillBatch, num_cus, ring_bpc);
}
inline uint32_t ring_fill_grid(uint32_t n, int num_cus, int ring_bpc)
{
    return batch_fill_grid(n, kGridRingBatch, num_cus, ring_bpc);
}

struct PieceGrid {
    uint32_t grid, ppb;
};
inline PieceGrid piece_fill_grid(uint32_t n, uint32_t max_length_hint, int num_cus, int fill_bpc)
{
    const uint32_t ppb = (uint32_t)(((uint64_t)max_length_hint + kGridFillPiece - 1) / kGridFillPiece);
    const uint64_t total = (uint64_t)n * ppb;
    const uint64_t cap = (uint64_t)num_cus * (uint64_t)(fill_bpc > 0 ? fill_bpc : 1);
    return PieceGrid{(uint32_t)(total < cap ? total : cap), ppb};
}

}
```

ctstraffic_amd/csrc/cts_internal.hpp:

```cpp
#pragma once

#include <hip/hip_runtime_api.h>
#include <stdint.h>

#include "cts_connections.h"
#include "cts_engine.h"
#include "cts_media_stream.h"
#include "cts_media_stream_conns.h"
#include "cts_media_stream_servers.h"
#include "cts_tcp_senders.h"

namespace cts {

constexpr int kCounterSlots = 8;
enum CounterSlot {
    kBytesChecked = 0,
    kBytesOk = 1,
    kBuffersChecked = 2,
    kBuffersFailed = 3,
    kMismatchedBytes = 4,
    kConnectionsFailed = 5
};
constexpr int kCounterCount = 6;
static_assert(kCounterCount <= kCounterSlots, "counters fit a shard line");

inline cts_counters_ex counters_ex_of(const uint64_t* v)
{
    return cts_counters_ex{v[kBytesChecked],  v[kBytesOk],         v[kBuffersChecked],
                           v[kBuffersFailed], v[kMismatchedBytes], v[kConnectionsFailed]};
}
inline cts_counters counters_of(const cts_counters_ex& x)
{
    return cts_counters{x.bytes_checked, x.bytes_ok, x.buffers_checked, x.buffers_failed, x.mismatched_bytes};
}

constexpr int kVerifyKernelId = 25;
constexpr int kSmallKernelId = 15;
constexpr int kMediaStreamKernelId = 3;

struct LaunchGeometry {
    int num_cus = 256;
    int blocks_per_cu = 4;
    int small_blocks_per_cu = 64;
    int nontemporal = 1;
    int small_threshold = 8192;
    int small_chunk = 0;
    int fill_nt = 2;
    int fill_blocks_per_cu = 1;
    int ring_fill_blocks_per_cu = 4;
};

struct alignas(64) MailSlot {
    uint64_t ptr_exp;
    uint64_t len_seq;
    uint64_t pad[6];
};
static_assert(sizeof(MailSlot) == 64, "one cache line per slot");
inline void mail_write(MailSlot* s, uint64_t ptr_exp, uint64_t len_seq)
{
    __atomic_store_n(&s->ptr_exp, ptr_exp, __ATOMIC_RELAXED);
    __atomic_store_n(&s->len_seq, len_seq, __ATOMIC_RELEASE);
}
struct alignas(16) MailPart {
    uint64_t g0;
    uint64_t g1;
};
constexpr uint32_t kMailPieceBytes = 4096;
#ifndef CTS_MAIL_GROUP
#define CTS_MAIL_GROUP 4
#endif
constexpr uint32_t kMailGroup = CTS_MAIL_GROUP;
#if defined(__HIP__)
__host__ __device__
#endif
inline uint32_t mail_parts(uint64_t ptr, uint32_t len)
{
    if (len == 0) return kMailGroup;
    const uint64_t pieces = (((ptr & 15u) + (uint64_t)len + 15u) / 16u * 16u + kMailPieceBytes - 1) / kMailPieceBytes;
    return pieces < kMailGroup ? (uint32_t)pieces : kMailGroup;
}
constexpr uint32_t kMailMaxGroups = 64;
constexpr uint32_t kMailSkip = 0xFFFFFFFFu;
struct MailStarts {
    uint64_t j[kMailMaxGroups];
};
hipError_t launch_mailbox(const MailSlot* slots, MailPart* parts, uint32_t per_group, const MailStarts& starts,
                          uint32_t groups, uint64_t idle_ticks, hipStream_t stream, uint64_t delay_ticks = 0);

hipError_t launch_counters_fold(const void* block, uint64_t* out, bool accumulate, hipStream_t stream);

hipError_t launch_verify(const uint8_t* arena, uint64_t arena_bytes, const cts_buf_desc* descs, uint32_t n,
                         uint32_t max_length_hint, cts_verify_result* results, uint64_t* counters,
                         uint32_t* conn_first_fail, uint32_t n_conns, hipStream_t stream,
                         const LaunchGeometry& geo);

hipError_t launch_verify_strided(const uint8_t* arena, uint64_t arena_bytes, uint32_t stride, const uint32_t* lens,
                                 uint32_t n, uint32_t skip_head, uint32_t expected, uint32_t conn_index,
                                 cts_verify_result* results, uint64_t* counters, uint32_t* conn_first_fail,
                                 uint32_t n_conns, hipStream_t stream, const LaunchGeometry& geo);

hipError_t launch_verify_at(const uint8_t* arena, uint64_t arena_bytes, const cts_buf_desc* descs, uint32_t n,
                            uint32_t max_length_hint, cts_verify_result* results, uint64_t* counters,
                            uint32_t* conn_first_fail, uint32_t n_conns, uint32_t base_index, hipStream_t stream,
                            const LaunchGeometry& geo);
hipError_t launch_verify_strided_at(const uint8_t* arena, uint64_t arena_bytes, uint32_t stride, const uint32_t* lens,
                                    uint32_t n, uint32_t skip_head, uint32_t expected, uint32_t conn_index,
                                    cts_verify_result* results, uint64_t* counters, uint32_t* conn_first_fail,
                                    uint32_t n_conns, uint32_t base_index, hipStream_t stream,
                                    const LaunchGeometry& geo);

hipError_t launch_refview(uint64_t arena_bytes, const cts_buf_desc* descs, uint32_t n, uint32_t base_index,
                          const uint32_t* conn_first_fail, uint32_t n_conns, uint64_t* ref_counters, hipStream_t stream,
                          const LaunchGeometry& geo);
hipError_t launch_refview_strided(uint64_t arena_bytes, uint32_t stride, const uint32_t* lens, uint32_t n,
                                  uint32_t skip_head, uint32_t conn_index, uint32_t base_index,
                                  const uint32_t* conn_first_fail, uint32_t n_conns, uint64_t* ref_counters,
                                  hipStream_t stream, const LaunchGeometry& geo);

hipError_t launch_conn_accumulate(uint64_t arena_bytes, const cts_buf_desc* descs, uint32_t n, uint32_t base_index,
                                  const uint32_t* conn_first_fail, uint32_t n_conns, uint64_t* ref_counters,
                                  cts_conn_state* conn_state, hipStream_t stream, const LaunchGeometry& geo);
hipError_t launch_conn_accumulate_strided(uint64_t arena_bytes, uint32_t stride, const uint32_t* lens, uint32_t n,
                                          uint32_t skip_head, uint32_t conn_index, uint32_t base_index,
                                          const uint32_t* conn_first_fail, uint32_t n_conns, uint64_t* ref_counters,
                                          cts_conn_state* conn_state, hipStream_t stream, const LaunchGeometry& geo);
hipError_t launch_conn_close(const uint32_t* conn_ids, const uint64_t* expected_bytes, uint32_t n,
                             uint32_t* conn_first_fail, cts_conn_state* conn_state, uint32_t n_conns,
                             cts_conn_result* results, uint64_t* close_counters, hipStream_t stream,
                             const LaunchGeometry& geo);
hipError_t launch_conn_slots_rebase(uint32_t* conn_first_fail, uint32_t n_conns, uint32_t delta, hipStream_t stream,
                                    const LaunchGeometry& geo);

hipError_t launch_media_stream_status_at(const uint8_t* arena, uint64_t arena_bytes, const cts_buf_desc* descs,
                                        uint32_t n, uint32_t base_index, cts_datagram_status* status,
                                        uint64_t* counters, uint32_t* conn_first_fail, uint32_t n_conns,
                                        hipStream_t stream, const LaunchGeometry& geo);
hipError_t launch_ms_conn_accumulate(const cts_buf_desc* descs, const cts_datagram_status* status, uint32_t n,
                                     uint32_t base_index, const uint32_t* conn_first_fail, cts_ms_conn_state* conns,
                                     uint64_t* frame_bytes, uint64_t frame_elems, uint32_t n_conns,
                                     uint64_t* udp_counters, hipStream_t stream, const LaunchGeometry& geo);
hipError_t launch_ms_conn_render(const uint32_t* conn_ids, uint32_t n, cts_ms_conn_state* conns, uint64_t* frame_bytes,
                                 uint32_t n_conns, uint64_t* udp_counters, uint32_t* codes, hipStream_t stream,
                                 const LaunchGeometry& geo);
hipError_t launch_ms_conn_close(const uint32_t* conn_ids, uint32_t n, uint32_t* conn_first_fail,
                                cts_ms_conn_state* conns, uint64_t* frame_bytes, uint32_t n_conns,
                                cts_ms_conn_result* results, uint64_t* close_counters, hipStream_t stream,
                                const LaunchGeometry& geo);

constexpr uint32_t kMsServerTile = 256;
inline uint64_t ms_server_tiles(uint32_t n) { return ((uint64_t)n + kMsServerTile - 1) / kMsServerTile; }
struct MsServerScratch {
    uint64_t* prefix;
    uint64_t* sums;
    cts_ms_server_tick* tick;
    MsServerScratch(void* base, uint32_t n)
        : prefix(static_cast<uint64_t*>(base)), sums(prefix + (uint64_t)n + 1),
          tick(reinterpret_cast<cts_ms_server_tick*>(sums + ms_server_tiles(n)))
    {
    }
    static size_t bytes(uint32_t n)
    {
        return (size_t)(((uint64_t)n + 1 + ms_server_tiles(n)) * sizeof(uint64_t) + sizeof(cts_ms_server_tick));
    }
};
hipError_t launch_ms_server_plan(const uint32_t* conn_ids, uint32_t n, cts_ms_server_state* servers, uint32_t n_conns,
                                 uint32_t stride, uint32_t capacity, uint32_t* codes, cts_ms_server_tick* tick,
                                 uint64_t* udp_counters, const MsServerScratch& scratch, hipStream_t stream);
hipError_t launch_ms_server_fill(uint8_t* arena, uint64_t arena_bytes, uint32_t stride, uint64_t first_slot,
                                 uint32_t capacity, const uint32_t* conn_ids, uint32_t n,
                                 const cts_ms_server_state* servers, uint32_t n_conns, const uint64_t* prefix,
                                 const cts_ms_server_tick* tick, int64_t qpc, int64_t qpf, cts_buf_desc* descs,
                                 uint32_t* lengths, hipStream_t stream, const LaunchGeometry& geo);

struct TcpSenderScratch {
    uint64_t* prefix;
    uint64_t* sums;
    uint64_t* before;
    cts_tcp_sender_tick* tick;
    TcpSenderScratch(void* base, uint32_t n)
        : prefix(static_cast<uint64_t*>(base)), sums(prefix + (uint64_t)n + 1), before(sums + ms_server_tiles(n)),
          tick(reinterpret_cast<cts_tcp_sender_tick*>(before + n))
    {
    }
    static size_t bytes(uint32_t n)
    {
        return (size_t)((2 * (uint64_t)n + 1 + ms_server_tiles(n)) * sizeof(uint64_t) + sizeof(cts_tcp_sender_tick));
    }
};
hipError_t launch_tcp_sender_plan(const uint32_t* conn_ids, uint32_t n, uint32_t max_buffers,
                                  cts_tcp_sender_state* senders, uint32_t n_conns, uint32_t stride, uint32_t capacity,
                                  uint32_t* codes, cts_tcp_sender_tick* tick, uint64_t* sent_counters,
                                  const TcpSenderScratch& scratch, hipStream_t stream);
hipError_t launch_tcp_sender_descs(uint32_t stride, uint64_t first_slot, uint32_t capacity, const uint32_t* conn_ids,
                                   uint32_t n, const cts_tcp_sender_state* senders, uint32_t n_conns,
                                   const TcpSenderScratch& scratch, const cts_tcp_sender_tick* tick,
                                   cts_buf_desc* descs, hipStream_t stream, const LaunchGeometry& geo);
hipError_t launch_tcp_sender_fill(uint8_t* arena, uint64_t arena_bytes, uint32_t stride, uint32_t capacity,
                                  const cts_buf_desc* descs, const cts_tcp_sender_tick* tick, hipStream_t stream,
                                  const LaunchGeometry& geo);

const LaunchGeometry& engine_geometry(const cts_engine* e, int* device);

hipError_t launch_fill(uint8_t* arena, uint64_t arena_bytes, const cts_buf_desc* descs, uint32_t n,
                       uint32_t max_length_hint, hipStream_t stream, const LaunchGeometry& geo);

hipError_t launch_fill_span(uint8_t* dst, uint64_t bytes, uint32_t pattern_offset, hipStream_t stream,
                            const LaunchGeometry& geo);

hipError_t launch_media_stream_verify(const uint8_t* arena, uint64_t arena_bytes, const cts_buf_desc* descs, uint32_t n,
                                     cts_datagram_record* records, cts_verify_result* results, uint64_t* counters,
                                     hipStream_t stream, const LaunchGeometry& geo);

hipError_t launch_media_stream_verify_strided(const uint8_t* arena, uint64_t arena_bytes, uint32_t stride,
                                             const uint32_t* lengths, uint32_t n, cts_datagram_record* records,
                                             cts_verify_result* results, uint64_t* counters, hipStream_t stream,
                                             const LaunchGeometry& geo);

hipError_t launch_media_stream_status(const uint8_t* arena, uint64_t arena_bytes, const cts_buf_desc* descs,
                                     const uint32_t* lengths, uint32_t stride, uint32_t n, cts_datagram_status* status,
                                     uint64_t* counters, hipStream_t stream, const LaunchGeometry& geo);

hipError_t launch_media_stream_frames(const uint8_t* arena, uint64_t arena_bytes, const cts_buf_desc* descs,
                                     const uint32_t* lengths, uint32_t stride, uint32_t n, const cts_frame_window& win,
                                     uint64_t* totals, uint64_t* frame_bytes, uint64_t* counters, hipStream_t stream,
                                     const LaunchGeometry& geo);

hipError_t launch_media_stream_fill(uint8_t* arena, uint64_t arena_bytes, const cts_buf_desc* descs,
                                   const cts_datagram_header* headers, uint32_t n, hipStream_t stream,
                                   const LaunchGeometry& geo);
hipError_t launch_media_stream_fill_strided(uint8_t* arena, uint64_t arena_bytes, uint32_t stride, const uint32_t* lengths,
                                           const cts_datagram_header* headers, uint32_t n, hipStream_t stream,
                                           const LaunchGeometry& geo);

}
```

ctstraffic_amd/csrc/cts_launch.hpp:

```cpp
#pragma once

#include <type_traits>

#include "cts_grids.hpp"
#include "cts_internal.hpp"

namespace cts {

inline uint32_t grid_for(uint32_t n, int teams_per_block, const LaunchGeometry& geo, int bpc_cap = 0)
{
    const int bpc = bpc_cap > 0 ? bpc_cap : (teams_per_block > 1 ? geo.small_blocks_per_cu : geo.blocks_per_cu);
    return grid_for(n, teams_per_block, geo.num_cus, bpc);
}

inline ContigGrid contig_grid(uint32_t n, const LaunchGeometry& geo)
{
    return contig_grid(n, geo.num_cus, geo.small_blocks_per_cu, geo.small_chunk);
}

template <bool... Bs, typename F>
inline void with_flags(F&& f)
{
    f(std::bool_constant<Bs>{}...);
}
template <bool... Bs, typename F, typename... Rest>
inline void with_flags(F&& f, bool flag, Rest... rest)
{
    if (flag) with_flags<Bs..., true>(f, rest...);
    else with_flags<Bs..., false>(f, rest...);
}

}
```

ctstraffic_amd/csrc/cts_media_stream_servers.cpp:

```cpp
#include <hip/hip_runtime_api.h>

#include "cts_internal.hpp"
#include "cts_media_stream_servers.h"

static_assert(sizeof(cts_ms_server_state) == 48 && alignof(cts_ms_server_state) == 8, "cts_ms_server_state: 48 bytes");
static_assert(sizeof(cts_ms_server_tick) == 32 && alignof(cts_ms_server_tick) == 8, "cts_ms_server_tick: 32 bytes");
static_assert(sizeof(cts_counters_udp) == 6 * sizeof(uint64_t), "a UDP block's six words are a counter block's");

namespace {

struct DeviceGuard {
    int prev = -1;
    bool ok = false;
    explicit DeviceGuard(int dev)
    {
        if (hipGetDevice(&prev) != hipSuccess) prev = -1;
        ok = (prev == dev) || (hipSetDevice(dev) == hipSuccess);
    }
    ~DeviceGuard()
    {
        if (prev >= 0) (void)hipSetDevice(prev);
    }
};

inline int hip_status(hipError_t e) { return e == hipSuccess ? CTS_OK : CTS_E_HIP; }

inline bool misaligned(const void* p, uintptr_t a) { return ((uintptr_t)p & (a - 1u)) != 0; }

}

extern "C" {

int cts_ms_server_init(const cts_media_stream_settings* s, cts_ms_server_state* out)
{
    if (s == nullptr || out == nullptr) return CTS_E_INVALID;
    if (s->frame_size_bytes <= CTS_UDP_DATA_HEADER_LENGTH) return CTS_E_INVALID;
    if (s->frames_per_second == 0 || s->stream_length_frames <= 0 || s->stream_length_frames > (int64_t)UINT32_MAX)
        return CTS_E_INVALID;
    if (s->datagram_max_size < CTS_MS_SERVER_MIN_DATAGRAM) return CTS_E_INVALID;
    *out = cts_ms_server_state{};
    out->current_frame = 1;
    out->final_frame = s->stream_length_frames;
    out->frame_size_bytes = s->frame_size_bytes;
    out->datagram_max_size = s->datagram_max_size;
    out->datagrams_per_frame =
        (uint32_t)(((uint64_t)s->frame_size_bytes + s->datagram_max_size - 1) / s->datagram_max_size);
    return CTS_OK;
}

size_t cts_media_stream_servers_scratch_bytes(uint32_t n) { return cts::MsServerScratch::bytes(n); }

int cts_media_stream_servers_send(cts_engine* e, void* dev_arena, uint64_t arena_bytes, uint32_t stride,
                                  uint64_t first_slot, uint32_t capacity, const uint32_t* dev_conn_ids, uint32_t n,
                                  cts_ms_server_state* dev_servers, uint32_t n_conns, int64_t qpc, int64_t qpf,
                                  cts_buf_desc* dev_descs, uint32_t* dev_lengths, uint32_t* dev_codes,
                                  cts_ms_server_tick* dev_tick, void* dev_udp_counters, void* dev_scratch,
                                  size_t scratch_bytes, void* stream)
{
    if (e == nullptr) return CTS_E_INVALID;
    if (n == 0) return CTS_OK;
    if ((stride & 15u) != 0u || stride < 32u || stride > (1u << 20)) return CTS_E_INVALID;
    if (dev_arena == nullptr || misaligned(dev_arena, 16)) return CTS_E_INVALID;
    if (first_slot > arena_bytes / stride || (uint64_t)capacity > arena_bytes / stride - first_slot)
        return CTS_E_INVALID;
    if (dev_conn_ids == nullptr || misaligned(dev_conn_ids, 4)) return CTS_E_INVALID;
    if ((n_conns != 0 && dev_servers == nullptr) || misaligned(dev_servers, 8)) return CTS_E_INVALID;
    if (misaligned(dev_descs, 8) || misaligned(dev_lengths, 4) || misaligned(dev_codes, 4) ||
        misaligned(dev_tick, 8) || misaligned(dev_udp_counters, 8))
        return CTS_E_INVALID;
    if (dev_scratch == nullptr || misaligned(dev_scratch, 8) || scratch_bytes < cts::MsServerScratch::bytes(n))
        return CTS_E_INVALID;
    int device = 0;
    const cts::LaunchGeometry& geo = cts::engine_geometry(e, &device);
    DeviceGuard g(device);
    if (!g.ok) return CTS_E_HIP;
    const cts::MsServerScratch scratch(dev_scratch, n);
    cts_ms_server_tick* const tick = dev_tick != nullptr ? dev_tick : scratch.tick;
    hipStream_t const s = static_cast<hipStream_t>(stream);
    const hipError_t rc = cts::launch_ms_server_plan(dev_conn_ids, n, dev_servers, n_conns, stride, capacity, dev_codes,
                                                     tick, static_cast<uint64_t*>(dev_udp_counters), scratch, s);
    if (rc != hipSuccess) return CTS_E_HIP;
    return hip_status(cts::launch_ms_server_fill(static_cast<uint8_t*>(dev_arena), arena_bytes, stride, first_slot,
                                                 capacity, dev_conn_ids, n, dev_servers, n_conns, scratch.prefix, tick,
                                                 qpc, qpf, dev_descs, dev_lengths, s, geo));
}

}
```

ctstraffic_amd/csrc/cts_tcp_senders.cpp:

```cpp
#include <hip/hip_runtime_api.h>

#include "cts_internal.hpp"
#include "cts_tcp_senders.h"

static_assert(sizeof(cts_tcp_sender_state) == 32 && alignof(cts_tcp_sender_state) == 8, "cts_tcp_sender_state: 32 bytes");
static_assert(sizeof(cts_tcp_sender_tick) == 32 && alignof(cts_tcp_sender_tick) == 8, "cts_tcp_sender_tick: 32 bytes");
static_assert(sizeof(cts_counters_sent) == 6 * sizeof(uint64_t), "a sent block's six words are a counter block's");

namespace {

struct DeviceGuard {
    int prev = -1;
    bool ok = false;
    explicit DeviceGuard(int dev)
    {
        if (hipGetDevice(&prev) != hipSuccess) prev = -1;
        ok = (prev == dev) || (hipSetDevice(dev) == hipSuccess);
    }
    ~DeviceGuard()
    {
        if (prev >= 0) (void)hipSetDevice(prev);
    }
};

inline int hip_status(hipError_t e) { return e == hipSuccess ? CTS_OK : CTS_E_HIP; }

inline bool misaligned(const void* p, uintptr_t a) { return ((uintptr_t)p & (a - 1u)) != 0; }

inline cts_counters_sent sent_of(const cts_counters_ex& x)
{
    return cts_counters_sent{x.bytes_checked, x.bytes_ok, x.buffers_checked, {0, 0, 0}};
}

}

extern "C" {

int cts_tcp_sender_init(uint64_t transfer_bytes, uint32_t buffer_size, cts_tcp_sender_state* out)
{
    if (out == nullptr || transfer_bytes == 0 || buffer_size == 0) return CTS_E_INVALID;
    *out = cts_tcp_sender_state{};
    out->transfer_bytes = transfer_bytes;
    out->buffer_size = buffer_size;
    return CTS_OK;
}

size_t cts_tcp_senders_scratch_bytes(uint32_t n) { return cts::TcpSenderScratch::bytes(n); }

int cts_tcp_senders_send(cts_engine* e, void* dev_arena, uint64_t arena_bytes, uint32_t stride, uint64_t first_slot,
                         uint32_t capacity, const uint32_t* dev_conn_ids, uint32_t n, uint32_t max_buffers,
                         cts_tcp_sender_state* dev_senders, uint32_t n_conns, cts_buf_desc* dev_descs,
                         uint32_t* dev_codes, cts_tcp_sender_tick* dev_tick, void* dev_sent_counters,
                         void* dev_scratch, size_t scratch_bytes, void* stream)
{
    if (e == nullptr) return CTS_E_INVALID;
    if (n == 0) return CTS_OK;
    if ((stride & 15u) != 0u || stride < 16u || stride > (16u << 20)) return CTS_E_INVALID;
    if (max_buffers == 0u) return CTS_E_INVALID;
    if (dev_arena == nullptr || misaligned(dev_arena, 16)) return CTS_E_INVALID;
    if (first_slot > arena_bytes / stride || (uint64_t)capacity > arena_bytes / stride - first_slot)
        return CTS_E_INVALID;
    if (dev_conn_ids == nullptr || misaligned(dev_conn_ids, 4)) return CTS_E_INVALID;
    if ((n_conns != 0 && dev_senders == nullptr) || misaligned(dev_senders, 8)) return CTS_E_INVALID;
    if (dev_descs == nullptr || misaligned(dev_descs, 8)) return CTS_E_INVALID;
    if (misaligned(dev_codes, 4) || misaligned(dev_tick, 8) || misaligned(dev_sent_counters, 8)) return CTS_E_INVALID;
    if (dev_scratch == nullptr || misaligned(dev_scratch, 8) || scratch_bytes < cts::TcpSenderScratch::bytes(n))
        return CTS_E_INVALID;
    int device = 0;
    const cts::LaunchGeometry& geo = cts::engine_geometry(e, &device);
    DeviceGuard g(device);
    if (!g.ok) return CTS_E_HIP;
    const cts::TcpSenderScratch scratch(dev_scratch, n);
    cts_tcp_sender_tick* const tick = dev_tick != nullptr ? dev_tick : scratch.tick;
    hipStream_t const s = static_cast<hipStream_t>(stream);
    hipError_t rc = cts::launch_tcp_sender_plan(dev_conn_ids, n, max_buffers, dev_senders, n_conns, stride, capacity,
                                                dev_codes, tick, static_cast<uint64_t*>(dev_sent_counters), scratch, s);
    if (rc != hipSuccess) return CTS_E_HIP;
    rc = cts::launch_tcp_sender_descs(stride, first_slot, capacity, dev_conn_ids, n, dev_senders, n_conns, scratch,
                                      tick, dev_descs, s, geo);
    if (rc != hipSuccess) return CTS_E_HIP;
    return hip_status(cts::launch_tcp_sender_fill(static_cast<uint8_t*>(dev_arena), arena_bytes, stride, capacity,
                                                  dev_descs, tick, s, geo));
}

int cts_counters_read_sent(cts_engine* e, const void* dev_sent_counters, cts_counters_sent* out, void* stream)
{
    if (out == nullptr) return CTS_E_INVALID;
    cts_counters_ex x{};
    const int rc = cts_counters_read_ex(e, dev_sent_counters, &x, stream);
    if (rc == CTS_OK) *out = sent_of(x);
    return rc;
}

int cts_counters_read_multi_sent(cts_engine* const* engines, const void* const* dev_sent_counters,
                                 void* const* streams, uint32_t n, cts_counters_sent* out)
{
    if (out == nullptr) return CTS_E_INVALID;
    cts_counters_ex x{};
    const int rc = cts_counters_read_multi_ex(engines, dev_sent_counters, streams, n, &x);
    if (rc == CTS_OK) *out = sent_of(x);
    return rc;
}

int cts_counters_allreduce_sent(cts_engine* const* engines, const void* const* dev_sent_counters,
                                void* const* streams, uint32_t n, cts_counters_sent* out)
{
    if (out == nullptr) return CTS_E_INVALID;
    cts_counters_ex x{};
    const int rc = cts_counters_allreduce_ex(engines, dev_sent_counters, streams, n, &x);
    if (rc == CTS_OK) *out = sent_of(x);
    return rc;
}

}
```

include/cts_engine.h:

```cpp
#ifndef CTS_ENGINE_H
#define CTS_ENGINE_H

#include <stddef.h>
#include <stdint.h>

#ifdef __cplusplus
extern "C" {
#endif

#define CTS_PATTERN_PERIOD 65536u
#define CTS_UDP_DATA_HEADER_LENGTH 26u
#define CTS_STATUS_ERROR_DATA_DID_NOT_MATCH_BIT_PATTERN 2147483644u
#define CTS_COUNTER_SHARDS 64u

typedef enum cts_status {
    CTS_OK = 0,
    CTS_E_INVALID = -1,
    CTS_E_HIP = -2,
    CTS_E_NOMEM = -3,
    CTS_E_NO_DEVICE = -4,
    CTS_E_UNAVAILABLE = -5,
    CTS_E_TIMEOUT = -6
} cts_status;

typedef struct cts_buf_desc {
    uint64_t byte_offset;
    uint32_t length;
    uint32_t expected_pattern_offset;
    uint32_t conn_index;
    uint32_t skip_head;
} cts_buf_desc;

#define CTS_RESULT_FLAG_BAD_DESC 0x1u

typedef struct cts_verify_result {
    uint32_t first_mismatch;
    uint32_t mismatch_bytes;
    uint8_t expected;
    uint8_t actual;
    uint8_t pass;
    uint8_t flags;
} cts_verify_result;

typedef struct cts_counters {
    uint64_t bytes_checked;
    uint64_t bytes_ok;
    uint64_t buffers_checked;
    uint64_t buffers_failed;
    uint64_t mismatched_bytes;
} cts_counters;

typedef struct cts_counters_ex {
    uint64_t bytes_checked;
    uint64_t bytes_ok;
    uint64_t buffers_checked;
    uint64_t buffers_failed;
    uint64_t mismatched_bytes;
    uint64_t connections_failed;
} cts_counters_ex;

typedef struct cts_counters_ref {
    uint64_t bytes_recv;
    uint64_t bytes_ok;
    uint64_t buffers_recv;
    uint64_t buffers_failed;
    uint64_t bytes_after_failure;
    uint64_t buffers_after_failure;
} cts_counters_ref;

typedef struct cts_engine cts_engine;

const char* cts_version(void);
const char* cts_status_string(int status);
uint8_t cts_pattern_byte(uint64_t stream_offset);
uint64_t cts_sender_buffer_size(uint32_t max_buffer_size);

uint32_t cts_shard_of(uint32_t conn_index, uint32_t n_shards);

int cts_engine_create(int device, cts_engine** out);
int cts_engine_destroy(cts_engine* engine);
int cts_engine_device(const cts_engine* engine);
int cts_engine_numa_node(const cts_engine* engine);

typedef enum cts_engine_attr {
    CTS_ATTR_BLOCKS_PER_CU = 1,
    CTS_ATTR_NT_LOADS = 2,
    CTS_ATTR_SMALL_THRESHOLD = 3,
    CTS_ATTR_VERIFY_VARIANT = 4,
    CTS_ATTR_SMALL_BLOCKS_PER_CU = 5,
    CTS_ATTR_SMALL_VARIANT = 6,
    CTS_ATTR_FILL_BLOCKS_PER_CU = 7,
    CTS_ATTR_MS_VARIANT = 8,
    CTS_ATTR_SMALL_CHUNK = 9,
    CTS_ATTR_FILL_NT = 10,
    CTS_ATTR_SYNC_MAILBOX = 11
} cts_engine_attr;
int cts_engine_set_attr(cts_engine* engine, int attr, int value);
int cts_engine_stream_create(cts_engine* engine, void** stream);
int cts_engine_stream_destroy(cts_engine* engine, void* stream);
int cts_engine_get_attr(const cts_engine* engine, int attr, int* value);

int cts_sender_buffer_fill(cts_engine* engine, void* dev_dst, uint32_t max_buffer_size, void* stream);

int cts_fill(cts_engine* engine, void* dev_arena, uint64_t arena_bytes,
             const cts_buf_desc* dev_descs, uint32_t n, uint32_t max_length_hint, void* stream);

int cts_verify(cts_engine* engine, const void* dev_arena, uint64_t arena_bytes,
               const cts_buf_desc* dev_descs, uint32_t n, uint32_t max_length_hint,
               cts_verify_result* dev_results, void* dev_counters,
               uint32_t* dev_conn_first_fail, uint32_t n_conns, void* stream);

size_t cts_counters_device_bytes(void);
int cts_counters_reset(cts_engine* engine, void* dev_counters, void* stream);
int cts_counters_read(cts_engine* engine, const void* dev_counters, cts_counters* out, void* stream);
int cts_counters_read_multi(cts_engine* const* engines, const void* const* dev_counters, void* const* streams,
                            uint32_t n, cts_counters* out);
int cts_counters_allreduce(cts_engine* const* engines, const void* const* dev_counters, void* const* streams,
                           uint32_t n, cts_counters* out);
int cts_counters_allreduce_release(void);

int cts_counters_read_ex(cts_engine* engine, const void* dev_counters, cts_counters_ex* out, void* stream);
int cts_counters_read_multi_ex(cts_engine* const* engines, const void* const* dev_counters, void* const* streams,
                               uint32_t n, cts_counters_ex* out);
int cts_counters_allreduce_ex(cts_engine* const* engines, const void* const* dev_counters, void* const* streams,
                              uint32_t n, cts_counters_ex* out);

int cts_counters_allreduce_prepare(cts_engine* const* engines, uint32_t n);

typedef struct cts_allreduce_setup {
    double rccl_load_ms;
    double slots_ms;
    double comm_init_ms;
    double first_allreduce_ms;
    uint32_t devices;
    uint32_t prepared;
    double last_fold_us;
    double last_allreduce_us;
    double last_readback_us;
    double last_total_us;
} cts_allreduce_setup;
int cts_counters_allreduce_setup_times(cts_allreduce_setup* out);

int cts_verify_strided(cts_engine* engine, const void* dev_arena, uint64_t arena_bytes, uint32_t stride,
                       const uint32_t* dev_lengths, uint32_t n, uint32_t skip_head, uint32_t expected_offset,
                       uint32_t conn_index, cts_verify_result* dev_results, void* dev_counters,
                       uint32_t* dev_conn_first_fail, uint32_t n_conns, void* stream);

int cts_verify_at(cts_engine* engine, const void* dev_arena, uint64_t arena_bytes, const cts_buf_desc* dev_descs,
                  uint32_t n, uint32_t max_length_hint, uint32_t base_index, cts_verify_result* dev_results,
                  void* dev_counters, uint32_t* dev_conn_first_fail, uint32_t n_conns, void* stream);
int cts_verify_strided_at(cts_engine* engine, const void* dev_arena, uint64_t arena_bytes, uint32_t stride,
                          const uint32_t* dev_lengths, uint32_t n, uint32_t skip_head, uint32_t expected_offset,
                          uint32_t conn_index, uint32_t base_index, cts_verify_result* dev_results,
                          void* dev_counters, uint32_t* dev_conn_first_fail, uint32_t n_conns, void* stream);

int cts_refview_accumulate(cts_engine* engine, uint64_t arena_bytes, const cts_buf_desc* dev_descs, uint32_t n,
                           uint32_t base_index, const uint32_t* dev_conn_first_fail, uint32_t n_conns,
                           void* dev_ref_counters, void* stream);
int cts_refview_accumulate_strided(cts_engine* engine, uint64_t arena_bytes, uint32_t stride,
                                   const uint32_t* dev_lengths, uint32_t n, uint32_t skip_head, uint32_t conn_index,
                                   uint32_t base_index, const uint32_t* dev_conn_first_fail, uint32_t n_conns,
                                   void* dev_ref_counters, void* stream);

int cts_counters_read_ref(cts_engine* engine, const void* dev_ref_counters, cts_counters_ref* out, void* stream);
int cts_counters_read_multi_ref(cts_engine* const* engines, const void* const* dev_ref_counters, void* const* streams,
                                uint32_t n, cts_counters_ref* out);
int cts_counters_allreduce_ref(cts_engine* const* engines, const void* const* dev_ref_counters, void* const* streams,
                               uint32_t n, cts_counters_ref* out);

int cts_verify_host(cts_engine* engine, const void* host_buf, uint32_t len,
                    uint32_t expected_offset, cts_verify_result* out);

int cts_verify_mapped(cts_engine* engine, const void* dev_buf, uint32_t len,
                      uint32_t expected_offset, cts_verify_result* out);
uint64_t cts_mailbox_launches(const cts_engine* engine);

int cts_host_alloc(cts_engine* engine, uint64_t bytes, void** host_ptr, void** dev_view);
int cts_host_free(cts_engine* engine, void* host_ptr);
int cts_host_device_pointer(void* host_ptr, void** dev_view);

int cts_verify_host_batch(cts_engine* engine, const void* const* bufs, const uint32_t* lens,
                          const uint32_t* expected, const uint32_t* skip_heads, uint32_t n,
                          cts_verify_result* results, cts_counters* counters);

#ifdef __cplusplus
}
#endif

#endif
```

Measured before the change: 6689.

## Add single-launch plan kernels for small media-stream and TCP sender ticks

For small connection counts (up to plan_one_max, default 1024), the per-tick plan uses one single-block kernel that loops over tiles with a carried prefix, replacing the separate sums, scan and apply launches. It can optionally also emit buffer descriptors in the same kernel, but that path is off by default. The aim is to cut kernel launch overhead and inter-kernel gaps on the control path. The cost is a serial single-block loop over connections. The main metric is bulk verify bandwidth, so this path may not touch it.

After: 6649. Within noise of the previous version (-0.6%).

```diff
diff --git a/ctstraffic_amd/_lib.py b/ctstraffic_amd/_lib.py
--- a/ctstraffic_amd/_lib.py
+++ b/ctstraffic_amd/_lib.py
@@ -36,6 +36,8 @@
 ATTR_SMALL_CHUNK = 9
 ATTR_FILL_NT = 10
 ATTR_SYNC_MAILBOX = 11
+ATTR_PLAN_ONE_MAX = 12
+ATTR_PLAN_ONE_DESC_MAX = 13
 
 
 VERIFY_KERNEL_ID = 25
diff --git a/ctstraffic_amd/csrc/cts_engine.cpp b/ctstraffic_amd/csrc/cts_engine.cpp
--- a/ctstraffic_amd/csrc/cts_engine.cpp
+++ b/ctstraffic_amd/csrc/cts_engine.cpp
@@ -516,6 +516,10 @@
     e->geo.small_chunk = env_int("CTS_SMALL_CHUNK", e->geo.small_chunk);
     e->geo.fill_nt = env_int("CTS_FILL_NT", e->geo.fill_nt);
     e->geo.ring_fill_blocks_per_cu = env_int("CTS_RING_FILL_BLOCKS_PER_CU", e->geo.ring_fill_blocks_per_cu);
+    e->geo.plan_one_max = env_int("CTS_PLAN_ONE_MAX", e->geo.plan_one_max);
+    e->geo.plan_one_desc_max = env_int("CTS_PLAN_ONE_DESC_MAX", e->geo.plan_one_desc_max);
+    if (e->geo.plan_one_max < 0) e->geo.plan_one_max = 0;
+    if (e->geo.plan_one_desc_max < 0) e->geo.plan_one_desc_max = 0;
     e->sync_mailbox = env_int("CTS_SYNC_MAILBOX", e->sync_mailbox) ? 1 : 0;
     if (hipStreamCreateWithFlags(&e->stream, hipStreamNonBlocking) != hipSuccess) {
         delete e;
@@ -630,6 +634,14 @@
     case CTS_ATTR_FILL_NT:
         if (value < 0 || value > 2) return CTS_E_INVALID;
         e->geo.fill_nt = value;
+        return CTS_OK;
+    case CTS_ATTR_PLAN_ONE_MAX:
+        if (value < 0) return CTS_E_INVALID;
+        e->geo.plan_one_max = value;
+        return CTS_OK;
+    case CTS_ATTR_PLAN_ONE_DESC_MAX:
+        if (value < 0) return CTS_E_INVALID;
+        e->geo.plan_one_desc_max = value;
         return CTS_OK;
     default: return CTS_E_INVALID;
     }
@@ -650,6 +662,8 @@
     case CTS_ATTR_SMALL_CHUNK: *value = e->geo.small_chunk; return CTS_OK;
     case CTS_ATTR_FILL_NT: *value = e->geo.fill_nt; return CTS_OK;
     case CTS_ATTR_SYNC_MAILBOX: *value = e->sync_mailbox; return CTS_OK;
+    case CTS_ATTR_PLAN_ONE_MAX: *value = e->geo.plan_one_max; return CTS_OK;
+    case CTS_ATTR_PLAN_ONE_DESC_MAX: *value = e->geo.plan_one_desc_max; return CTS_OK;
     default: return CTS_E_INVALID;
     }
 }
diff --git a/ctstraffic_amd/csrc/cts_fill.hip b/ctstraffic_amd/csrc/cts_fill.hip
--- a/ctstraffic_amd/csrc/cts_fill.hip
+++ b/ctstraffic_amd/csrc/cts_fill.hip
@@ -392,57 +392,59 @@
     if (threadIdx.x < sizeof(cts_ms_server_tick) / 4u) tick[threadIdx.x] = 0u;
 }
 
-__global__ void __launch_bounds__(kBlock)
-    ms_server_apply(const uint32_t* __restrict__ ids, uint32_t n, cts_ms_server_state* __restrict__ servers,
-                    uint32_t n_conns, uint32_t stride, uint32_t capacity, const uint64_t* __restrict__ sums,
-                    uint64_t* __restrict__ prefix, uint32_t* __restrict__ codes, cts_ms_server_tick* __restrict__ tick,
-                    uint64_t* __restrict__ udp)
-{
-    __shared__ uint64_t wsum[kBlock / 64];
-    __shared__ uint64_t ctr[kBlock / 64][kCounterCount];
-    __shared__ uint32_t red[kBlock / 64][5];
-    zero_counters<kBlock / 64>(ctr);
-    const uint64_t i = (uint64_t)blockIdx.x * kMsServerTile + threadIdx.x;
-    uint32_t code = CTS_MS_SERVER_SENT, c = 0u;
-    uint64_t want = 0;
-    if (i < n) {
-        c = ids[i];
-        want = ms_server_want(servers, c, n_conns, stride, code);
-    }
-    uint64_t total;
-    const uint64_t p = sums[blockIdx.x] + tile_scan_exclusive(want, wsum, total);
+struct MsServerLaneSums {
     uint64_t bytes = 0;
     uint32_t datagrams = 0, sent = 0, finished = 0, no_room = 0, skipped = 0;
-    if (i < n) {
-        prefix[i] = p;
-        if (code != CTS_MS_SERVER_SENT) {
-            skipped = 1u;
-        } else if (p + want > (uint64_t)capacity) {
-            no_room = 1u;
-            code = CTS_MS_SERVER_NO_ROOM;
-        } else {
-            cts_ms_server_state* e = servers + c;
-            bytes = e->frame_size_bytes;
-            datagrams = (uint32_t)want;
-            sent = 1u;
-            e->bits_sent += 8u * bytes;
-            e->datagrams_sent += want;
-            const int64_t next = e->current_frame + 1;
-            e->current_frame = next;
-            if (next > e->final_frame) {
-                e->finished = 1u;
-                finished = 1u;
-                code = CTS_MS_SERVER_FINISHED;
-            }
-        }
-        if (codes != nullptr) codes[i] = code;
-    }
-    bytes = wave_sum64(bytes);
-    datagrams = wave_sum(datagrams);
-    sent = wave_sum(sent);
-    finished = wave_sum(finished);
-    no_room = wave_sum(no_room);
-    skipped = wave_sum(skipped);
+};
+
+__device__ __forceinline__ uint64_t ms_server_want_of(const cts_ms_server_state& e, bool valid, uint32_t stride,
+                                                      uint32_t& code)
+{
+    const bool ended = e.finished != 0u, fits = e.datagram_max_size <= stride;
+    code = !valid ? CTS_MS_SERVER_SKIPPED : ended ? CTS_MS_SERVER_ENDED : fits ? CTS_MS_SERVER_SENT : CTS_MS_SERVER_SKIPPED;
+    return code == CTS_MS_SERVER_SENT ? (uint64_t)e.datagrams_per_frame : 0u;
+}
+
+__device__ __forceinline__ void ms_server_lane(uint64_t i, uint32_t c, const cts_ms_server_state& ev, uint64_t want,
+                                               uint32_t code, uint64_t p, cts_ms_server_state* __restrict__ servers,
+                                               uint32_t capacity, uint64_t* __restrict__ prefix,
+                                               uint32_t* __restrict__ codes, MsServerLaneSums& a)
+{
+    prefix[i] = p;
+    if (code != CTS_MS_SERVER_SENT) {
+        a.skipped += 1u;
+    } else if (p + want > (uint64_t)capacity) {
+        a.no_room += 1u;
+        code = CTS_MS_SERVER_NO_ROOM;
+    } else {
+        cts_ms_server_state* e = servers + c;
+        const uint64_t bytes = ev.frame_size_bytes;
+        a.bytes += bytes;
+        a.datagrams += (uint32_t)want;
+        a.sent += 1u;
+        e->bits_sent = ev.bits_sent + 8u * bytes;
+        e->datagrams_sent = ev.datagrams_sent + want;
+        const int64_t next = ev.current_frame + 1;
+        e->current_frame = next;
+        if (next > ev.final_frame) {
+            e->finished = 1u;
+            a.finished += 1u;
+            code = CTS_MS_SERVER_FINISHED;
+        }
+    }
+    if (codes != nullptr) codes[i] = code;
+}
+
+__device__ __forceinline__ void ms_server_reduce(const MsServerLaneSums& a, uint64_t (*ctr)[kCounterCount],
+                                                 uint32_t (*red)[5], cts_ms_server_tick* __restrict__ tick,
+                                                 uint64_t* __restrict__ udp)
+{
+    const uint64_t bytes = wave_sum64(a.bytes);
+    const uint32_t datagrams = wave_sum(a.datagrams);
+    const uint32_t sent = wave_sum(a.sent);
+    const uint32_t finished = wave_sum(a.finished);
+    const uint32_t no_room = wave_sum(a.no_room);
+    const uint32_t skipped = wave_sum(a.skipped);
     const uint32_t wave = threadIdx.x >> 6;
     if ((threadIdx.x & 63u) == 0u) {
         ctr[wave][0] = 8u * bytes;
@@ -466,6 +468,65 @@
         for (int w = 0; w < kBlock / 64; ++w) s += ctr[w][0];
         if (s) atomicAdd((unsigned long long*)&tick->bytes, (unsigned long long)(s / 8u));
     }
+}
+
+__global__ void __launch_bounds__(kBlock)
+    ms_server_apply(const uint32_t* __restrict__ ids, uint32_t n, cts_ms_server_state* __restrict__ servers,
+                    uint32_t n_conns, uint32_t stride, uint32_t capacity, const uint64_t* __restrict__ sums,
+                    uint64_t* __restrict__ prefix, uint32_t* __restrict__ codes, cts_ms_server_tick* __restrict__ tick,
+                    uint64_t* __restrict__ udp)
+{
+    __shared__ uint64_t wsum[kBlock / 64];
+    __shared__ uint64_t ctr[kBlock / 64][kCounterCount];
+    __shared__ uint32_t red[kBlock / 64][5];
+    zero_counters<kBlock / 64>(ctr);
+    const uint64_t i = (uint64_t)blockIdx.x * kMsServerTile + threadIdx.x;
+    uint32_t code = CTS_MS_SERVER_SKIPPED, c = 0u;
+    cts_ms_server_state ev = {};
+    uint64_t want = 0;
+    if (i < n) {
+        c = ids[i];
+        if (c < n_conns) ev = servers[c];
+        want = ms_server_want_of(ev, c < n_conns, stride, code);
+    }
+    uint64_t total;
+    const uint64_t p = sums[blockIdx.x] + tile_scan_exclusive(want, wsum, total);
+    MsServerLaneSums a;
+    if (i < n) ms_server_lane(i, c, ev, want, code, p, servers, capacity, prefix, codes, a);
+    ms_server_reduce(a, ctr, red, tick, udp);
+}
+
+__global__ void __launch_bounds__(kBlock)
+    ms_server_plan_one(const uint32_t* __restrict__ ids, uint32_t n, cts_ms_server_state* __restrict__ servers,
+                       uint32_t n_conns, uint32_t stride, uint32_t capacity, uint64_t* __restrict__ prefix,
+                       uint32_t* __restrict__ codes, cts_ms_server_tick* __restrict__ tick, uint64_t* __restrict__ udp)
+{
+    __shared__ uint64_t wsum[kBlock / 64];
+    __shared__ uint64_t ctr[kBlock / 64][kCounterCount];
+    __shared__ uint32_t red[kBlock / 64][5];
+    if (threadIdx.x < sizeof(cts_ms_server_tick) / 4u) reinterpret_cast<uint32_t*>(tick)[threadIdx.x] = 0u;
+    zero_counters<kBlock / 64>(ctr);
+    const uint32_t none = 0xFFFFFFFFu;
+    uint32_t c = threadIdx.x < n ? ids[threadIdx.x] : none;
+    uint32_t c_next = (uint64_t)threadIdx.x + kMsServerTile < n ? ids[threadIdx.x + kMsServerTile] : none;
+    cts_ms_server_state ev = {};
+    if (c < n_conns) ev = servers[c];
+    uint64_t carry = 0;
+    MsServerLaneSums a;
+    for (uint64_t i = threadIdx.x; i - threadIdx.x < n; i += kMsServerTile) {
+        cts_ms_server_state ev_next = {};
+        if (c_next < n_conns) ev_next = servers[c_next];
+        const uint32_t c_after = i + 2u * kMsServerTile < n ? ids[i + 2u * kMsServerTile] : none;
+        uint32_t code;
+        const uint64_t want = ms_server_want_of(ev, c < n_conns, stride, code);
+        uint64_t total;
+        const uint64_t p = carry + tile_scan_exclusive(i < n ? want : 0u, wsum, total);
+        if (i < n) ms_server_lane(i, c, ev, want, code, p, servers, capacity, prefix, codes, a);
+        carry += total;
+        c = c_next, c_next = c_after, ev = ev_next;
+    }
+    if (threadIdx.x == 0u) prefix[n] = carry;
+    ms_server_reduce(a, ctr, red, tick, udp);
 }
 
 __device__ __forceinline__ uint64_t ms_server_listed(const uint64_t* __restrict__ prefix, uint64_t lo, uint64_t hi,
@@ -598,61 +659,69 @@
     }
 }
 
-__global__ void __launch_bounds__(kBlock)
-    tcp_sender_apply(const uint32_t* __restrict__ ids, uint32_t n, cts_tcp_sender_state* __restrict__ senders,
-                     uint32_t n_conns, uint32_t stride, uint32_t capacity, uint32_t max_buffers,
-                     const uint64_t* __restrict__ sums, uint64_t* __restrict__ prefix, uint64_t* __restrict__ before,
-                     uint32_t* __restrict__ codes, cts_tcp_sender_tick* __restrict__ tick, uint64_t* __restrict__ sent_block)
-{
-    __shared__ uint64_t wsum[kBlock / 64];
-    __shared__ uint64_t ctr[kBlock / 64][kCounterCount];
-    __shared__ uint32_t red[kBlock / 64][5];
-    zero_counters<kBlock / 64>(ctr);
-    const uint64_t i = (uint64_t)blockIdx.x * kMsServerTile + threadIdx.x;
-    uint32_t code = CTS_TCP_SENDER_SENT, c = 0u;
-    uint64_t want = 0;
-    if (i < n) {
-        c = ids[i];
-        want = tcp_sender_want(senders, c, n_conns, stride, max_buffers, code);
-    }
-    uint64_t total;
-    const uint64_t p = sums[blockIdx.x] + tile_scan_exclusive(want, wsum, total);
+struct TcpSenderLaneSums {
     uint64_t bytes = 0;
     uint32_t buffers = 0, sent = 0, finished = 0, no_room = 0, skipped = 0;
-    if (i < n) {
-        prefix[i] = p;
-        const uint64_t pc = p < (uint64_t)capacity ? p : (uint64_t)capacity;
-        const uint64_t t = want < (uint64_t)capacity - pc ? want : (uint64_t)capacity - pc;
-        uint64_t was = 0;
-        if (code != CTS_TCP_SENDER_SENT) {
-            skipped = 1u;
-        } else if (t == 0u) {
-            no_room = 1u;
-            code = CTS_TCP_SENDER_NO_ROOM;
-        } else {
-            cts_tcp_sender_state* e = senders + c;
-            was = e->bytes_sent;
-            const uint64_t R = e->transfer_bytes - was, full = t * e->buffer_size;
-            bytes = full < R ? full : R;
-            buffers = (uint32_t)t;
-            sent = 1u;
-            e->bytes_sent = was + bytes;
-            e->buffers_sent += t;
-            if (bytes == R) {
-                e->finished = 1u;
-                finished = 1u;
-                code = CTS_TCP_SENDER_FINISHED;
-            }
-        }
-        before[i] = was;
-        if (codes != nullptr) codes[i] = code;
-    }
-    const uint64_t own_bytes = tcp_wave_sum64(bytes);
-    buffers = wave_sum(buffers);
-    sent = wave_sum(sent);
-    finished = wave_sum(finished);
-    no_room = wave_sum(no_room);
-    skipped = wave_sum(skipped);
+};
+
+__device__ __forceinline__ uint64_t tcp_sender_want_of(const cts_tcp_sender_state& e, bool valid, uint32_t stride,
+                                                       uint32_t max_buffers, uint32_t& code)
+{
+    const uint32_t B = e.buffer_size;
+    const bool usable = valid && B != 0u && B <= stride;
+    const bool running = e.finished == 0u && e.bytes_sent < e.transfer_bytes;
+    code = !usable ? CTS_TCP_SENDER_SKIPPED : running ? CTS_TCP_SENDER_SENT : CTS_TCP_SENDER_ENDED;
+    if (code != CTS_TCP_SENDER_SENT) return 0u;
+    const uint64_t R = e.transfer_bytes - e.bytes_sent;
+    const uint64_t k = R / B + (R % B != 0u ? 1u : 0u);
+    return k < max_buffers ? k : max_buffers;
+}
+
+__device__ __forceinline__ void tcp_sender_lane(uint64_t i, uint32_t c, const cts_tcp_sender_state& ev, uint64_t want,
+                                                uint32_t code, uint64_t p, cts_tcp_sender_state* __restrict__ senders,
+                                                uint32_t capacity, uint64_t* __restrict__ prefix,
+                                                uint64_t* __restrict__ before, uint32_t* __restrict__ codes,
+                                                TcpSenderLaneSums& a)
+{
+    prefix[i] = p;
+    const uint64_t pc = p < (uint64_t)capacity ? p : (uint64_t)capacity;
+    const uint64_t t = want < (uint64_t)capacity - pc ? want : (uint64_t)capacity - pc;
+    uint64_t was = 0;
+    if (code != CTS_TCP_SENDER_SENT) {
+        a.skipped += 1u;
+    } else if (t == 0u) {
+        a.no_room += 1u;
+        code = CTS_TCP_SENDER_NO_ROOM;
+    } else {
+        cts_tcp_sender_state* e = senders + c;
+        was = ev.bytes_sent;
+        const uint64_t R = ev.transfer_bytes - was, full = t * ev.buffer_size;
+        const uint64_t bytes = full < R ? full : R;
+        a.bytes += bytes;
+        a.buffers += (uint32_t)t;
+        a.sent += 1u;
+        e->bytes_sent = was + bytes;
+        e->buffers_sent = ev.buffers_sent + t;
+        if (bytes == R) {
+            e->finished = 1u;
+            a.finished += 1u;
+            code = CTS_TCP_SENDER_FINISHED;
+        }
+    }
+    before[i] = was;
+    if (codes != nullptr) codes[i] = code;
+}
+
+__device__ __forceinline__ void tcp_sender_reduce(const TcpSenderLaneSums& a, uint64_t (*ctr)[kCounterCount],
+                                                  uint32_t (*red)[5], cts_tcp_sender_tick* __restrict__ tick,
+                                                  uint64_t* __restrict__ sent_block)
+{
+    const uint64_t own_bytes = tcp_wave_sum64(a.bytes);
+    const uint32_t buffers = wave_sum(a.buffers);
+    const uint32_t sent = wave_sum(a.sent);
+    const uint32_t finished = wave_sum(a.finished);
+    const uint32_t no_room = wave_sum(a.no_room);
+    const uint32_t skipped = wave_sum(a.skipped);
     const uint32_t wave = threadIdx.x >> 6;
     if ((threadIdx.x & 63u) == 0u) {
         ctr[wave][0] = own_bytes;
@@ -680,6 +749,46 @@
 }
 
 __global__ void __launch_bounds__(kBlock)
+    tcp_sender_apply(const uint32_t* __restrict__ ids, uint32_t n, cts_tcp_sender_state* __restrict__ senders,
+                     uint32_t n_conns, uint32_t stride, uint32_t capacity, uint32_t max_buffers,
+                     const uint64_t* __restrict__ sums, uint64_t* __restrict__ prefix, uint64_t* __restrict__ before,
+                     uint32_t* __restrict__ codes, cts_tcp_sender_tick* __restrict__ tick, uint64_t* __restrict__ sent_block)
+{
+    __shared__ uint64_t wsum[kBlock / 64];
+    __shared__ uint64_t ctr[kBlock / 64][kCounterCount];
+    __shared__ uint32_t red[kBlock / 64][5];
+    zero_counters<kBlock / 64>(ctr);
+    const uint64_t i = (uint64_t)blockIdx.x * kMsServerTile + threadIdx.x;
+    uint32_t code = CTS_TCP_SENDER_SKIPPED, c = 0u;
+    cts_tcp_sender_state ev = {};
+    uint64_t want = 0;
+    if (i < n) {
+        c = ids[i];
+        if (c < n_conns) ev = senders[c];
+        want = tcp_sender_want_of(ev, c < n_conns, stride, max_buffers, code);
+    }
+    uint64_t total;
+    const uint64_t p = sums[blockIdx.x] + tile_scan_exclusive(want, wsum, total);
+    TcpSenderLaneSums a;
+    if (i < n) tcp_sender_lane(i, c, ev, want, code, p, senders, capacity, prefix, before, codes, a);
+    tcp_sender_reduce(a, ctr, red, tick, sent_block);
+}
+
+__device__ __forceinline__ cts_buf_desc tcp_sender_desc(uint64_t g, uint64_t j, uint32_t c, bool valid, uint64_t was,
+                                                        uint32_t B, uint64_t end, uint32_t stride, uint64_t first_slot)
+{
+    uint32_t len = 0u, off = 0u;
+    if (valid) {
+        const uint64_t start = was + j * B;
+        const uint64_t left = start < end ? end - start : 0u;
+        len = left < (uint64_t)B ? (uint32_t)left : B;
+        if (len > stride) len = 0u;
+        off = (uint32_t)(start & 0xFFFFu);
+    }
+    return cts_buf_desc{(first_slot + g) * stride, len, off, c, 0u};
+}
+
+__global__ void __launch_bounds__(kBlock)
     tcp_sender_descs(uint32_t stride, uint64_t first_slot, uint32_t capacity, const uint32_t* __restrict__ ids,
                      uint32_t n, const cts_tcp_sender_state* __restrict__ senders, uint32_t n_conns,
                      const uint64_t* __restrict__ prefix, const uint64_t* __restrict__ before,
@@ -690,17 +799,103 @@
         const uint64_t i = ms_server_listed(prefix, 0u, n, g);
         const uint64_t j = g - prefix[i];
         const uint32_t c = ids[i];
-        uint32_t len = 0u, off = 0u;
+        uint32_t B = 0u;
+        uint64_t was = 0u, end = 0u;
         if (c < n_conns) {
-            const uint32_t B = senders[c].buffer_size;
-            const uint64_t was = before[i], start = was + j * B;
-            const uint64_t end = senders[c].transfer_bytes;
-            const uint64_t left = start < end ? end - start : 0u;
-            len = left < (uint64_t)B ? (uint32_t)left : B;
-            if (len > stride) len = 0u;
-            off = (uint32_t)(start & 0xFFFFu);
-        }
-        descs[g] = cts_buf_desc{(first_slot + g) * stride, len, off, c, 0u};
+            B = senders[c].buffer_size;
+            was = before[i];
+            end = senders[c].transfer_bytes;
+        }
+        descs[g] = tcp_sender_desc(g, j, c, c < n_conns, was, B, end, stride, first_slot);
+    }
+}
+
+constexpr uint32_t kPlanOneSlots = 16;
+static_assert(kPlanOneLdsListed == kGridPlanOneLdsListed, "cts_grids.hpp sizes the list of a one-launch descriptor pass");
+
+template <bool DESCS>
+__global__ void __launch_bounds__(kBlock)
+    tcp_sender_plan_one(const uint32_t* __restrict__ ids, uint32_t n, cts_tcp_sender_state* __restrict__ senders,
+                        uint32_t n_conns, uint32_t stride, uint32_t capacity, uint32_t max_buffers,
+                        uint64_t* __restrict__ prefix, uint64_t* __restrict__ before, uint32_t* __restrict__ codes,
+                        cts_tcp_sender_tick* __restrict__ tick, uint64_t* __restrict__ sent_block, uint64_t first_slot,
+                        cts_buf_desc* __restrict__ descs)
+{
+    __shared__ uint64_t wsum[kBlock / 64];
+    __shared__ uint64_t ctr[kBlock / 64][kCounterCount];
+    __shared__ uint32_t red[kBlock / 64][5];
+    __shared__ uint32_t pfx[DESCS ? kPlanOneLdsListed : 1u];
+    if (threadIdx.x < sizeof(cts_tcp_sender_tick) / 4u) reinterpret_cast<uint32_t*>(tick)[threadIdx.x] = 0u;
+    zero_counters<kBlock / 64>(ctr);
+    const uint32_t none = 0xFFFFFFFFu;
+    uint32_t c = threadIdx.x < n ? ids[threadIdx.x] : none;
+    uint32_t c_next = (uint64_t)threadIdx.x + kMsServerTile < n ? ids[threadIdx.x + kMsServerTile] : none;
+    cts_tcp_sender_state ev = {};
+    if (c < n_conns) ev = senders[c];
+    uint64_t carry = 0;
+    TcpSenderLaneSums a;
+    for (uint64_t i = threadIdx.x; i - threadIdx.x < n; i += kMsServerTile) {
+        cts_tcp_sender_state ev_next = {};
+        if (c_next < n_conns) ev_next = senders[c_next];
+        const uint32_t c_after = i + 2u * kMsServerTile < n ? ids[i + 2u * kMsServerTile] : none;
+        uint32_t code;
+        const uint64_t want = tcp_sender_want_of(ev, c < n_conns, stride, max_buffers, code);
+        uint64_t total;
+        const uint64_t p = carry + tile_scan_exclusive(i < n ? want : 0u, wsum, total);
+        if (i < n) {
+            tcp_sender_lane(i, c, ev, want, code, p, senders, capacity, prefix, before, codes, a);
+            if constexpr (DESCS) pfx[i] = (uint32_t)(p < (uint64_t)capacity ? p : (uint64_t)capacity);
+        }
+        carry += total;
+        c = c_next, c_next = c_after, ev = ev_next;
+    }
+    if (threadIdx.x == 0u) prefix[n] = carry;
+    tcp_sender_reduce(a, ctr, red, tick, sent_block);
+    if constexpr (DESCS) {
+        __syncthreads();
+        uint32_t buffers = 0;
+#pragma unroll
+        for (int w = 0; w < kBlock / 64; ++w) buffers += red[w][0];
+        const uint32_t total = buffers < capacity ? buffers : capacity;
+        for (uint32_t g0 = threadIdx.x; g0 < total; g0 += kPlanOneSlots * kBlock) {
+            uint32_t gs[kPlanOneSlots], lo[kPlanOneSlots], hi[kPlanOneSlots];
+#pragma unroll
+            for (uint32_t k = 0; k < kPlanOneSlots; ++k) {
+                const uint32_t g = g0 + k * kBlock;
+                gs[k] = g < total ? g : total - 1u;
+                lo[k] = 0u;
+                hi[k] = n;
+            }
+            for (uint32_t span = n; span > 1u; span = (span + 1u) >> 1) {
+#pragma unroll
+                for (uint32_t k = 0; k < kPlanOneSlots; ++k) {
+                    const uint32_t mid = (lo[k] + hi[k]) >> 1;
+                    const bool le = pfx[mid] <= gs[k];
+                    lo[k] = le ? mid : lo[k];
+                    hi[k] = le ? hi[k] : mid;
+                }
+            }
+            uint32_t cs[kPlanOneSlots], Bs[kPlanOneSlots];
+            uint64_t was[kPlanOneSlots], ends[kPlanOneSlots];
+#pragma unroll
+            for (uint32_t k = 0; k < kPlanOneSlots; ++k) {
+                cs[k] = ids[lo[k]];
+                was[k] = before[lo[k]];
+            }
+#pragma unroll
+            for (uint32_t k = 0; k < kPlanOneSlots; ++k) {
+                const cts_tcp_sender_state* e = senders + (cs[k] < n_conns ? cs[k] : 0u);
+                Bs[k] = e->buffer_size;
+                ends[k] = e->transfer_bytes;
+            }
+#pragma unroll
+            for (uint32_t k = 0; k < kPlanOneSlots; ++k) {
+                const uint32_t g = g0 + k * kBlock;
+                if (g < total)
+                    descs[g] = tcp_sender_desc(g, (uint64_t)(g - pfx[lo[k]]), cs[k], cs[k] < n_conns, was[k], Bs[k],
+                                               ends[k], stride, first_slot);
+            }
+        }
     }
 }
 
@@ -787,9 +982,15 @@
 
 hipError_t launch_ms_server_plan(const uint32_t* conn_ids, uint32_t n, cts_ms_server_state* servers, uint32_t n_conns,
                                  uint32_t stride, uint32_t capacity, uint32_t* codes, cts_ms_server_tick* tick,
-                                 uint64_t* udp_counters, const MsServerScratch& scratch, hipStream_t stream)
+                                 uint64_t* udp_counters, const MsServerScratch& scratch, hipStream_t stream,
+                                 const LaunchGeometry& geo)
 {
     if (n == 0) return hipSuccess;
+    if (tick_plan_form(n, capacity, geo) != kPlanThreeLaunches) {
+        ms_server_plan_one<<<1, kBlock, 0, stream>>>(conn_ids, n, servers, n_conns, stride, capacity, scratch.prefix,
+                                                     codes, tick, udp_counters);
+        return hipGetLastError();
+    }
     const uint64_t tiles = ms_server_tiles(n);
     ms_server_sums<<<(uint32_t)tiles, kBlock, 0, stream>>>(conn_ids, n, servers, n_conns, stride, scratch.sums);
     ms_server_scan<<<1, kBlock, 0, stream>>>(scratch.sums, tiles, scratch.prefix + n,
@@ -825,11 +1026,23 @@
 }
 
 hipError_t launch_tcp_sender_plan(const uint32_t* conn_ids, uint32_t n, uint32_t max_buffers,
-                                  cts_tcp_sender_state* senders, uint32_t n_conns, uint32_t stride, uint32_t capacity,
-                                  uint32_t* codes, cts_tcp_sender_tick* tick, uint64_t* sent_counters,
-                                  const TcpSenderScratch& scratch, hipStream_t stream)
+                                  cts_tcp_sender_state* senders, uint32_t n_conns, uint32_t stride, uint64_t first_slot,
+                                  uint32_t capacity, uint32_t* codes, cts_tcp_sender_tick* tick, uint64_t* sent_counters,
+                                  cts_buf_desc* descs, const TcpSenderScratch& scratch, hipStream_t stream,
+                                  const LaunchGeometry& geo)
 {
     if (n == 0) return hipSuccess;
+    const int form = tick_plan_form(n, capacity, geo);
+    if (form != kPlanThreeLaunches) {
+        with_flags(
+            [&](auto DESCS) {
+                tcp_sender_plan_one<DESCS.value><<<1, kBlock, 0, stream>>>(
+                    conn_ids, n, senders, n_conns, stride, capacity, max_buffers, scratch.prefix, scratch.before, codes,
+                    tick, sent_counters, first_slot, descs);
+            },
+            form == kPlanOneLaunchDescs);
+        return hipGetLastError();
+    }
     const uint64_t tiles = ms_server_tiles(n);
     tcp_sender_sums<<<(uint32_t)tiles, kBlock, 0, stream>>>(conn_ids, n, senders, n_conns, stride, max_buffers,
                                                             scratch.sums);
@@ -847,6 +1060,7 @@
                                    cts_buf_desc* descs, hipStream_t stream, const LaunchGeometry& geo)
 {
     if (n == 0 || capacity == 0) return hipSuccess;
+    if (tick_plan_form(n, capacity, geo) == kPlanOneLaunchDescs) return hipSuccess;
     const uint32_t grid = grid_for((uint32_t)(((uint64_t)capacity + kBlock - 1) / kBlock), 1, geo);
     tcp_sender_descs<<<grid, kBlock, 0, stream>>>(stride, first_slot, capacity, conn_ids, n, senders, n_conns,
                                                   scratch.prefix, scratch.before, tick, descs);
diff --git a/ctstraffic_amd/csrc/cts_grids.hpp b/ctstraffic_amd/csrc/cts_grids.hpp
--- a/ctstraffic_amd/csrc/cts_grids.hpp
+++ b/ctstraffic_amd/csrc/cts_grids.hpp
@@ -62,4 +62,13 @@
     return PieceGrid{(uint32_t)(total < cap ? total : cap), ppb};
 }
 
+constexpr uint32_t kGridPlanOneLdsListed = 4096;
+enum TickPlanForm { kPlanThreeLaunches = 0, kPlanOneLaunch = 1, kPlanOneLaunchDescs = 2 };
+inline int tick_plan_form(uint32_t n, uint32_t capacity, uint32_t plan_one_max, uint32_t plan_one_desc_max)
+{
+    if (n == 0 || n > plan_one_max) return kPlanThreeLaunches;
+    if (capacity == 0 || capacity > plan_one_desc_max || n > kGridPlanOneLdsListed) return kPlanOneLaunch;
+    return kPlanOneLaunchDescs;
 }
+
+}
diff --git a/ctstraffic_amd/csrc/cts_internal.hpp b/ctstraffic_amd/csrc/cts_internal.hpp
--- a/ctstraffic_amd/csrc/cts_internal.hpp
+++ b/ctstraffic_amd/csrc/cts_internal.hpp
@@ -48,6 +48,8 @@
     int fill_nt = 2;
     int fill_blocks_per_cu = 1;
     int ring_fill_blocks_per_cu = 4;
+    int plan_one_max = 1024;
+    int plan_one_desc_max = 0;
 };
 
 struct alignas(64) MailSlot {
@@ -165,7 +167,8 @@
 };
 hipError_t launch_ms_server_plan(const uint32_t* conn_ids, uint32_t n, cts_ms_server_state* servers, uint32_t n_conns,
                                  uint32_t stride, uint32_t capacity, uint32_t* codes, cts_ms_server_tick* tick,
-                                 uint64_t* udp_counters, const MsServerScratch& scratch, hipStream_t stream);
+                                 uint64_t* udp_counters, const MsServerScratch& scratch, hipStream_t stream,
+                                 const LaunchGeometry& geo);
 hipError_t launch_ms_server_fill(uint8_t* arena, uint64_t arena_bytes, uint32_t stride, uint64_t first_slot,
                                  uint32_t capacity, const uint32_t* conn_ids, uint32_t n,
                                  const cts_ms_server_state* servers, uint32_t n_conns, const uint64_t* prefix,
@@ -187,10 +190,12 @@
         return (size_t)((2 * (uint64_t)n + 1 + ms_server_tiles(n)) * sizeof(uint64_t) + sizeof(cts_tcp_sender_tick));
     }
 };
+constexpr uint32_t kPlanOneLdsListed = 4096;
 hipError_t launch_tcp_sender_plan(const uint32_t* conn_ids, uint32_t n, uint32_t max_buffers,
-                                  cts_tcp_sender_state* senders, uint32_t n_conns, uint32_t stride, uint32_t capacity,
-                                  uint32_t* codes, cts_tcp_sender_tick* tick, uint64_t* sent_counters,
-                                  const TcpSenderScratch& scratch, hipStream_t stream);
+                                  cts_tcp_sender_state* senders, uint32_t n_conns, uint32_t stride, uint64_t first_slot,
+                                  uint32_t capacity, uint32_t* codes, cts_tcp_sender_tick* tick, uint64_t* sent_counters,
+                                  cts_buf_desc* descs, const TcpSenderScratch& scratch, hipStream_t stream,
+                                  const LaunchGeometry& geo);
 hipError_t launch_tcp_sender_descs(uint32_t stride, uint64_t first_slot, uint32_t capacity, const uint32_t* conn_ids,
                                    uint32_t n, const cts_tcp_sender_state* senders, uint32_t n_conns,
                                    const TcpSenderScratch& scratch, const cts_tcp_sender_tick* tick,
diff --git a/ctstraffic_amd/csrc/cts_launch.hpp b/ctstraffic_amd/csrc/cts_launch.hpp
--- a/ctstraffic_amd/csrc/cts_launch.hpp
+++ b/ctstraffic_amd/csrc/cts_launch.hpp
@@ -18,6 +18,12 @@
     return contig_grid(n, geo.num_cus, geo.small_blocks_per_cu, geo.small_chunk);
 }
 
+inline int tick_plan_form(uint32_t n, uint32_t capacity, const LaunchGeometry& geo)
+{
+    return tick_plan_form(n, capacity, (uint32_t)(geo.plan_one_max > 0 ? geo.plan_one_max : 0),
+                          (uint32_t)(geo.plan_one_desc_max > 0 ? geo.plan_one_desc_max : 0));
+}
+
 template <bool... Bs, typename F>
 inline void with_flags(F&& f)
 {
diff --git a/ctstraffic_amd/csrc/cts_media_stream_servers.cpp b/ctstraffic_amd/csrc/cts_media_stream_servers.cpp
--- a/ctstraffic_amd/csrc/cts_media_stream_servers.cpp
+++ b/ctstraffic_amd/csrc/cts_media_stream_servers.cpp
@@ -78,7 +78,7 @@
     cts_ms_server_tick* const tick = dev_tick != nullptr ? dev_tick : scratch.tick;
     hipStream_t const s = static_cast<hipStream_t>(stream);
     const hipError_t rc = cts::launch_ms_server_plan(dev_conn_ids, n, dev_servers, n_conns, stride, capacity, dev_codes,
-                                                     tick, static_cast<uint64_t*>(dev_udp_counters), scratch, s);
+                                                     tick, static_cast<uint64_t*>(dev_udp_counters), scratch, s, geo);
     if (rc != hipSuccess) return CTS_E_HIP;
     return hip_status(cts::launch_ms_server_fill(static_cast<uint8_t*>(dev_arena), arena_bytes, stride, first_slot,
                                                  capacity, dev_conn_ids, n, dev_servers, n_conns, scratch.prefix, tick,
diff --git a/ctstraffic_amd/csrc/cts_tcp_senders.cpp b/ctstraffic_amd/csrc/cts_tcp_senders.cpp
--- a/ctstraffic_amd/csrc/cts_tcp_senders.cpp
+++ b/ctstraffic_amd/csrc/cts_tcp_senders.cpp
@@ -73,8 +73,9 @@
     const cts::TcpSenderScratch scratch(dev_scratch, n);
     cts_tcp_sender_tick* const tick = dev_tick != nullptr ? dev_tick : scratch.tick;
     hipStream_t const s = static_cast<hipStream_t>(stream);
-    hipError_t rc = cts::launch_tcp_sender_plan(dev_conn_ids, n, max_buffers, dev_senders, n_conns, stride, capacity,
-                                                dev_codes, tick, static_cast<uint64_t*>(dev_sent_counters), scratch, s);
+    hipError_t rc = cts::launch_tcp_sender_plan(dev_conn_ids, n, max_buffers, dev_senders, n_conns, stride, first_slot,
+                                                capacity, dev_codes, tick, static_cast<uint64_t*>(dev_sent_counters),
+                                                dev_descs, scratch, s, geo);
     if (rc != hipSuccess) return CTS_E_HIP;
     rc = cts::launch_tcp_sender_descs(stride, first_slot, capacity, dev_conn_ids, n, dev_senders, n_conns, scratch,
                                       tick, dev_descs, s, geo);
diff --git a/include/cts_engine.h b/include/cts_engine.h
--- a/include/cts_engine.h
+++ b/include/cts_engine.h
@@ -93,7 +93,9 @@
     CTS_ATTR_MS_VARIANT = 8,
     CTS_ATTR_SMALL_CHUNK = 9,
     CTS_ATTR_FILL_NT = 10,
-    CTS_ATTR_SYNC_MAILBOX = 11
+    CTS_ATTR_SYNC_MAILBOX = 11,
+    CTS_ATTR_PLAN_ONE_MAX = 12,
+    CTS_ATTR_PLAN_ONE_DESC_MAX = 13
 } cts_engine_attr;
 int cts_engine_set_attr(cts_engine* engine, int attr, int value);
 int cts_engine_stream_create(cts_engine* engine, void** stream);
```
